# szabodabo/CUDA-MPI-Reductions

Hardware: AMD Instinct MI355X
Metric: reduction bandwidth (GB/s, whole node), 1B-double sum at 1/2/4/8 MI355X (higher is better)
Workload: dtype fp64; 1 GPU; global_batch=1000000000, seq_len=1, parallelism=dp1, backend=nccl, n_total_elements=1000000000, op=SUM, collective=fused, launch=graph (chunk 871, 1 replays)

## Files before the change

### csrc/kernels/direct.hip

```cpp
#include <hip/hip_runtime.h>

#include <algorithm>
#include <cstdint>
#include <cstring>

#include "mireduce/check.hpp"
#include "mireduce/device.hpp"
#include "mireduce/direct.hpp"
#include "mireduce/peer.hpp"
#include "mireduce/ops.hpp"

namespace mireduce {
namespace kern {

__device__ __forceinline__ void peer_barrier(const DirectDesc* d, int phase, unsigned e, unsigned err,
                                             bool release) {
  asm volatile("s_waitcnt vmcnt(0)" ::: "memory");
  __syncthreads();
  if (threadIdx.x < 64) {
    const int lane = threadIdx.x;
    if (release) __builtin_amdgcn_fence(__ATOMIC_RELEASE, "");
    const int world = d->world;
    const uint64_t slot = (static_cast<uint64_t>(phase) * kMaxDirectBlocks + blockIdx.x) * kMaxDirectRanks;
    if (lane < world) {
      __hip_atomic_store(d->sig[lane] + slot + d->rank, e, __ATOMIC_RELAXED, __HIP_MEMORY_SCOPE_SYSTEM);
      const unsigned* mine = d->sig[d->rank] + slot + lane;
      const uint64_t limit = err ? 0 : d->timeout_ticks;
      const uint64_t t0 = static_cast<uint64_t>(wall_clock64());
      while (__hip_atomic_load(mine, __ATOMIC_RELAXED, __HIP_MEMORY_SCOPE_SYSTEM) != e) {
        if (static_cast<uint64_t>(wall_clock64()) - t0 > limit) {
          __hip_atomic_fetch_or(d->ctl + 1, 1u, __ATOMIC_RELAXED, __HIP_MEMORY_SCOPE_AGENT);
          break;
        }
        __builtin_amdgcn_s_sleep(1);
      }
    }
    __builtin_amdgcn_fence(__ATOMIC_ACQUIRE, "");
  }
  __syncthreads();
}

__device__ __forceinline__ void block_range(uint64_t nvec, uint64_t* v0, uint64_t* v1) {
  const uint64_t per = (nvec + gridDim.x - 1) / gridDim.x;
  *v0 = std::min<uint64_t>(nvec, blockIdx.x * per);
  *v1 = std::min<uint64_t>(nvec, *v0 + per);
}

template <class T>
__device__ __forceinline__ uint64_t chunk_elems(uint64_t count, int world) {
  constexpr uint64_t N = 16 / sizeof(T);
  const uint64_t per = (count + world - 1) / world;
  return (per + N - 1) / N * N;
}

template <int W>
constexpr int direct_unroll() {
  return W >= 4 ? 1 : (W >= 2 ? 2 : 4);
}

template <class OpT, class T, int W>
__global__ __launch_bounds__(kDirectBlock) void direct_kernel(const DirectDesc* __restrict__ d, uint64_t count,
                                                               int gather_rank) {
  constexpr int N = 16 / sizeof(T);
  constexpr int U = W > 0 ? direct_unroll<W>() : 1;
  using V = T __attribute__((ext_vector_type(N)));
  __shared__ unsigned s_epoch, s_err;
  if (threadIdx.x == 0) {
    s_epoch = __hip_atomic_load(d->ctl, __ATOMIC_RELAXED, __HIP_MEMORY_SCOPE_AGENT) + 1u;
    s_err = __hip_atomic_load(d->ctl + 1, __ATOMIC_RELAXED, __HIP_MEMORY_SCOPE_AGENT);
  }
  __syncthreads();
  const unsigned e = s_epoch;
  const int world = W > 0 ? W : d->world;
  const int rank = d->rank;

  peer_barrier(d, 0, e, s_err, true);

  const uint64_t per = chunk_elems<T>(count, world);
  const uint64_t perv = per / N;
  uint64_t v0, v1;
  block_range(perv, &v0, &v1);
  {
    const uint64_t cb = std::min<uint64_t>(count, rank * per);
    const uint64_t ce = std::min<uint64_t>(count, cb + per);
    const uint64_t nvec = (ce - cb) / N;
    const uint64_t r1 = std::min(v1, nvec);
    T* out = reinterpret_cast<T*>(d->out[rank]);
    if constexpr (W > 0) {
      for (uint64_t i0 = v0 + threadIdx.x; i0 < r1; i0 += U * kDirectBlock) {
        V v[U][W];
#pragma unroll
        for (int u = 0; u < U; ++u) {
          const uint64_t i = i0 + static_cast<uint64_t>(u) * kDirectBlock;
          if (i < r1)
#pragma unroll
            for (int p = 0; p < W; ++p)
              v[u][p] = __builtin_nontemporal_load(reinterpret_cast<const V*>(d->in[p]) + cb / N + i);
        }
#pragma unroll
        for (int u = 0; u < U; ++u) {
          const uint64_t i = i0 + static_cast<uint64_t>(u) * kDirectBlock;
          if (i >= r1) continue;
          V acc = v[u][0];
#pragma unroll
          for (int p = 1; p < W; ++p)
#pragma unroll
            for (int k = 0; k < N; ++k) acc[k] = OpT::apply(acc[k], v[u][p][k]);
          reinterpret_cast<V*>(out)[cb / N + i] = acc;
        }
      }
    } else {
      for (uint64_t i = v0 + threadIdx.x; i < r1; i += kDirectBlock) {
        const uint64_t off = cb / N + i;
        V acc = __builtin_nontemporal_load(reinterpret_cast<const V*>(d->in[0]) + off);
        for (int p = 1; p < world; ++p) {
          const V v = __builtin_nontemporal_load(reinterpret_cast<const V*>(d->in[p]) + off);
#pragma unroll
          for (int k = 0; k < N; ++k) acc[k] = OpT::apply(acc[k], v[k]);
        }
        reinterpret_cast<V*>(out)[off] = acc;
      }
    }
    if (blockIdx.x == gridDim.x - 1) {
      for (uint64_t i = cb + nvec * N + threadIdx.x; i < ce; i += kDirectBlock) {
        T acc = reinterpret_cast<const T*>(d->in[0])[i];
        for (int p = 1; p < world; ++p) acc = OpT::apply(acc, reinterpret_cast<const T*>(d->in[p])[i]);
        out[i] = acc;
      }
    }
  }

  peer_barrier(d, 1, e, s_err, true);

  if (gather_rank < 0 || gather_rank == rank) {
    T* mine = reinterpret_cast<T*>(d->out[rank]);
    if constexpr (W > 0) {
      uint64_t nv[W];
#pragma unroll
      for (int p = 0; p < W; ++p) {
        const uint64_t b = std::min<uint64_t>(count, p * per);
        nv[p] = p == rank ? 0 : (std::min<uint64_t>(count, b + per) - b) / N;
      }
      for (uint64_t i0 = v0 + threadIdx.x; i0 < v1; i0 += U * kDirectBlock) {
        V v[U][W];
#pragma unroll
        for (int u = 0; u < U; ++u) {
          const uint64_t i = i0 + static_cast<uint64_t>(u) * kDirectBlock;
#pragma unroll
          for (int p = 0; p < W; ++p)
            if (i < v1 && i < nv[p])
              v[u][p] = __builtin_nontemporal_load(reinterpret_cast<const V*>(d->out[p]) + p * perv + i);
        }
#pragma unroll
        for (int u = 0; u < U; ++u) {
          const uint64_t i = i0 + static_cast<uint64_t>(u) * kDirectBlock;
#pragma unroll
          for (int p = 0; p < W; ++p)
            if (i < v1 && i < nv[p]) reinterpret_cast<V*>(mine)[p * perv + i] = v[u][p];
        }
      }
    } else {
      for (int p = 0; p < world; ++p) {
        if (p == rank) continue;
        const uint64_t b = std::min<uint64_t>(count, p * per);
        const uint64_t n = (std::min<uint64_t>(count, b + per) - b) / N;
        const uint64_t e1 = std::min(v1, n);
        for (uint64_t i = v0 + threadIdx.x; i < e1; i += kDirectBlock)
          reinterpret_cast<V*>(mine)[p * perv + i] = __builtin_nontemporal_load(reinterpret_cast<const V*>(d->out[p]) + p * perv + i);
      }
    }
    if (blockIdx.x == gridDim.x - 1) {
      for (int p = 0; p < world; ++p) {
        if (p == rank) continue;
        const uint64_t b = std::min<uint64_t>(count, p * per);
        const uint64_t e1 = std::min<uint64_t>(count, b + per);
        for (uint64_t i = b + (e1 - b) / N * N + threadIdx.x; i < e1; i += kDirectBlock)
          mine[i] = reinterpret_cast<const T*>(d->out[p])[i];
      }
    }
  }

  peer_barrier(d, 2, e, s_err, false);
  if (threadIdx.x == 0) {
    const unsigned prev = __hip_atomic_fetch_add(d->ctl + 2, 1u, __ATOMIC_RELAXED, __HIP_MEMORY_SCOPE_AGENT);
    if (prev == gridDim.x - 1) {
      __hip_atomic_store(d->ctl + 2, 0u, __ATOMIC_RELAXED, __HIP_MEMORY_SCOPE_AGENT);
      __hip_atomic_store(d->ctl, e, __ATOMIC_RELAXED, __HIP_MEMORY_SCOPE_AGENT);
    }
  }
}

}

void direct_chunk(size_t count, size_t elem_size, int world, int r, size_t* begin, size_t* end) {
  const size_t vec = 16 / elem_size;
  size_t per = (count + world - 1) / world;
  per = (per + vec - 1) / vec * vec;
  *begin = std::min(count, static_cast<size_t>(r) * per);
  *end = std::min(count, static_cast<size_t>(r + 1) * per);
}

namespace {

constexpr size_t kSigBytes = static_cast<size_t>(kDirectPhases) * kMaxDirectBlocks * kMaxDirectRanks * sizeof(unsigned);

using DirectFn = void (*)(const DirectDesc*, uint64_t, int, int, hipStream_t);

template <class OpT, class T, int W>
void launch_w(const DirectDesc* d, uint64_t count, int gather, int grid, hipStream_t s) {
  hipLaunchKernelGGL((kern::direct_kernel<OpT, T, W>), dim3(grid), dim3(kDirectBlock), 0, s, d, count, gather);
}

template <class OpT, class T>
DirectFn pick_world(int world) {
  switch (world) {
    case 1: return launch_w<OpT, T, 1>;
    case 2: return launch_w<OpT, T, 2>;
    case 3: return launch_w<OpT, T, 3>;
    case 4: return launch_w<OpT, T, 4>;
    case 5: return launch_w<OpT, T, 5>;
    case 6: return launch_w<OpT, T, 6>;
    case 7: return launch_w<OpT, T, 7>;
    case 8: return launch_w<OpT, T, 8>;
    default: return launch_w<OpT, T, 0>;
  }
}

template <class OpT>
DirectFn pick_type(DType t, int world) {
  switch (t) {
    case DType::Int32: return pick_world<OpT, int32_t>(world);
    case DType::Int64: return pick_world<OpT, int64_t>(world);
    case DType::Float32: return pick_world<OpT, float>(world);
    case DType::Float64: return pick_world<OpT, double>(world);
    default: MIREDUCE_REQUIRE(false, "direct: int32, int64, float32 or float64 only");
  }
  return nullptr;
}

}

DirectAllreduce::DirectAllreduce(int device, size_t bytes, int grid, double timeout_s) : timeout_s_(timeout_s) {
  MIREDUCE_REQUIRE(timeout_s > 0, "direct: timeout must be positive");
  if (device < 0) MIREDUCE_HIP_THROW(hipGetDevice(&device));
  device_ = device;
  DeviceGuard g(device_);
  grid_ = grid > 0 ? grid : device_cus(device_);
  MIREDUCE_REQUIRE(grid_ <= kMaxDirectBlocks, "direct: grid exceeds kMaxDirectBlocks");
  bytes_ = (std::max<size_t>(bytes, 16) + 255) / 256 * 256;
  MIREDUCE_HIP_THROW(hipExtMallocWithFlags(&in_, bytes_, hipDeviceMallocFinegrained));
  MIREDUCE_HIP_THROW(hipExtMallocWithFlags(&out_, bytes_, hipDeviceMallocFinegrained));
  MIREDUCE_HIP_THROW(hipExtMallocWithFlags(reinterpret_cast<void**>(&sig_), kSigBytes, hipDeviceMallocUncached));
  MIREDUCE_HIP_THROW(hipMemset(sig_, 0, kSigBytes));
  MIREDUCE_HIP_THROW(hipMalloc(reinterpret_cast<void**>(&ctl_), 256));
  MIREDUCE_HIP_THROW(hipMemset(ctl_, 0, 256));
  MIREDUCE_HIP_THROW(hipMalloc(reinterpret_cast<void**>(&desc_), sizeof(DirectDesc)));
  MIREDUCE_HIP_THROW(hipDeviceSynchronize());
}

DirectAllreduce::~DirectAllreduce() {
  DeviceGuard g(device_);
  for (void* p : opened_) (void)hipIpcCloseMemHandle(p);
  (void)hipFree(sink_);
  (void)hipFree(desc_);
  (void)hipFree(ctl_);
  (void)hipFree(sig_);
  (void)hipFree(out_);
  (void)hipFree(in_);
  (void)hipGetLastError();
}

std::vector<char> DirectAllreduce::handles() const {
  std::vector<char> h(kHandleBytes);
  void* bufs[3] = {in_, out_, sig_};
  for (int k = 0; k < 3; ++k) {
    hipIpcMemHandle_t m;
    MIREDUCE_HIP_THROW(hipIpcGetMemHandle(&m, bufs[k]));
    std::memcpy(h.data() + k * sizeof(IpcHandleBytes), &m, sizeof m);
  }
  const int32_t gr = grid_;
  std::memcpy(h.data() + 3 * sizeof(IpcHandleBytes), &gr, sizeof gr);
  return h;
}

void DirectAllreduce::connect(int rank, int world, const std::vector<std::vector<char>>& all) {
  MIREDUCE_REQUIRE(!connected_, "direct: already connected");
  MIREDUCE_REQUIRE(world >= 1 && world <= kMaxDirectRanks, "direct: world must be 1..16");
  MIREDUCE_REQUIRE(rank >= 0 && rank < world, "direct: rank out of range");
  MIREDUCE_REQUIRE(all.size() == static_cast<size_t>(world), "direct: one handle set per rank");
  DeviceGuard g(device_);
  DirectDesc d{};
  for (int r = 0; r < world; ++r) {
    MIREDUCE_REQUIRE(all[r].size() == kHandleBytes, "direct: bad handle size");
    int32_t gr = 0;
    std::memcpy(&gr, all[r].data() + 3 * sizeof(IpcHandleBytes), sizeof gr);
    MIREDUCE_REQUIRE(gr == grid_, "direct: every rank must use the same grid");
    if (r == rank) {
      d.in[r] = static_cast<const char*>(in_);
      d.out[r] = static_cast<char*>(out_);
      d.sig[r] = sig_;
      continue;
    }
    void* p[3] = {nullptr, nullptr, nullptr};
    for (int k = 0; k < 3; ++k) {
      hipIpcMemHandle_t m;
      std::memcpy(&m, all[r].data() + k * sizeof(IpcHandleBytes), sizeof m);
      MIREDUCE_HIP_THROW(hipIpcOpenMemHandle(&p[k], m, hipIpcMemLazyEnablePeerAccess));
      opened_.push_back(p[k]);
    }
    d.in[r] = static_cast<const char*>(p[0]);
    peer_in_.push_back(p[0]);
    d.out[r] = static_cast<char*>(p[1]);
    d.sig[r] = static_cast<unsigned*>(p[2]);
  }
  d.ctl = ctl_;
  d.rank = rank;
  d.world = world;
  int khz = 0;
  if (hipDeviceGetAttribute(&khz, hipDeviceAttributeWallClockRate, device_) != hipSuccess || khz <= 0) khz = 100000;
  d.timeout_ticks = static_cast<uint64_t>(timeout_s_ * 1e3 * khz);
  MIREDUCE_HIP_THROW(hipMemcpy(desc_, &d, sizeof d, hipMemcpyHostToDevice));
  MIREDUCE_HIP_THROW(hipDeviceSynchronize());
  rank_ = rank;
  world_ = world;
  connected_ = true;
}

void DirectAllreduce::launch(size_t count, DType t, Op op, int gather_rank, hipStream_t s) {
  MIREDUCE_REQUIRE(connected_, "direct: connect() first");
  MIREDUCE_REQUIRE(count * dtype_size(t) <= bytes_, "direct: count exceeds the registered buffers");
  DirectFn fn = nullptr;
  switch (op) {
    case Op::Sum: fn = pick_type<SumOp>(t, world_); break;
    case Op::Min: fn = pick_type<MinOp>(t, world_); break;
    case Op::Max: fn = pick_type<MaxOp>(t, world_); break;
    default: MIREDUCE_REQUIRE(false, "direct: SUM, MIN or MAX");
  }
  (void)hipGetLastError();
  fn(desc_, count, gather_rank, grid_, s);
  MIREDUCE_HIP_THROW(hipGetLastError());
}

void DirectAllreduce::allreduce(size_t count, DType t, Op op, hipStream_t s) { launch(count, t, op, -1, s); }

void DirectAllreduce::reduce(size_t count, DType t, Op op, int root, hipStream_t s) {
  MIREDUCE_REQUIRE(root >= 0 && root < world_, "direct: root out of range");
  launch(count, t, op, root, s);
}

void DirectAllreduce::read_peers(size_t bytes_each, hipStream_t s) {
  MIREDUCE_REQUIRE(connected_, "direct: connect() first");
  MIREDUCE_REQUIRE(bytes_each <= bytes_, "direct: read_peers beyond the registered buffers");
  DeviceGuard g(device_);
  PeerSources src{};
  int n = 0;
  if (peer_in_.empty()) src.p[n++] = in_;
  for (const void* p : peer_in_) src.p[n++] = p;
  const int grid = 128 * n;
  if (!sink_) MIREDUCE_HIP_THROW(hipMalloc(reinterpret_cast<void**>(&sink_), 128 * kMaxPeerSources * sizeof(uint32_t)));
  peer_read(src, n, bytes_each, sink_, grid, s);
}

unsigned DirectAllreduce::error() const {
  unsigned v = 0;
  DeviceGuard g(device_);
  MIREDUCE_HIP_THROW(hipMemcpy(&v, ctl_ + 1, sizeof v, hipMemcpyDeviceToHost));
  return v;
}

unsigned DirectAllreduce::epoch() const {
  unsigned v = 0;
  DeviceGuard g(device_);
  MIREDUCE_HIP_THROW(hipMemcpy(&v, ctl_, sizeof v, hipMemcpyDeviceToHost));
  return v;
}

}
```

Before: 7359 GB/s.

## Software-pipeline direct reduce and gather loops with global nontemporal tiles; skip barriers at world 1

Rewrites the reduce-scatter and gather phases of the direct kernel so that full tiles go through a double-buffered load/store loop. It uses explicit global address-space nontemporal loads and stores and places sched barriers so the next tile's loads are issued before the current tile's stores. This replaces flat, predicated, vmcnt(0)-serialised accesses. For a single rank it drops all three peer barriers and the gather phase. Range helpers move into a shared header, and reference assembly dumps are added. Risks are extra register pressure at large world sizes and nontemporal stores changing cache behaviour for readers of the output.

```diff
diff --git a/csrc/kernels/direct.hip b/csrc/kernels/direct.hip
--- a/csrc/kernels/direct.hip
+++ b/csrc/kernels/direct.hip
@@ -9,6 +9,8 @@
 #include "mireduce/direct.hpp"
 #include "mireduce/peer.hpp"
 #include "mireduce/ops.hpp"
+
+#include "direct_ranges.hpp"
 
 namespace mireduce {
 namespace kern {
@@ -40,22 +42,50 @@
   __syncthreads();
 }
 
-__device__ __forceinline__ void block_range(uint64_t nvec, uint64_t* v0, uint64_t* v1) {
-  const uint64_t per = (nvec + gridDim.x - 1) / gridDim.x;
-  *v0 = std::min<uint64_t>(nvec, blockIdx.x * per);
-  *v1 = std::min<uint64_t>(nvec, *v0 + per);
-}
-
-template <class T>
-__device__ __forceinline__ uint64_t chunk_elems(uint64_t count, int world) {
-  constexpr uint64_t N = 16 / sizeof(T);
-  const uint64_t per = (count + world - 1) / world;
-  return (per + N - 1) / N * N;
-}
-
 template <int W>
 constexpr int direct_unroll() {
   return W >= 4 ? 1 : (W >= 2 ? 2 : 4);
+}
+
+template <class V>
+using GlobalPtr = V __attribute__((address_space(1)))*;
+
+template <class V>
+__device__ __forceinline__ V ld_global_nt(const char* base, uint32_t off) {
+  return __builtin_nontemporal_load((GlobalPtr<const V>)(base + off));
+}
+template <class V>
+__device__ __forceinline__ void st_global(char* base, uint32_t off, V v) {
+  __builtin_nontemporal_store(v, (GlobalPtr<V>)(base + off));
+}
+
+template <class Set, class Load, class Store>
+__device__ __forceinline__ void stream_full_tiles(uint64_t nfull, Load load, Store store) {
+  if (nfull == 0) return;
+  __builtin_amdgcn_s_waitcnt(0);
+  Set a, b;
+  load(a, uint64_t{0});
+  uint64_t k = 0;
+#pragma clang loop unroll(disable)
+  for (; k + 2 < nfull; k += 2) {
+    load(b, k + 1);
+    __builtin_amdgcn_sched_barrier(0);
+    store(a, k);
+    __builtin_amdgcn_sched_barrier(0);
+    load(a, k + 2);
+    __builtin_amdgcn_sched_barrier(0);
+    store(b, k + 1);
+    __builtin_amdgcn_sched_barrier(0);
+  }
+  if (k + 1 < nfull) {
+    load(b, k + 1);
+    __builtin_amdgcn_sched_barrier(0);
+    store(a, k);
+    __builtin_amdgcn_sched_barrier(0);
+    store(b, k + 1);
+  } else {
+    store(a, k);
+  }
 }
 
 template <class OpT, class T, int W>
@@ -63,7 +93,10 @@
                                                                int gather_rank) {
   constexpr int N = 16 / sizeof(T);
   constexpr int U = W > 0 ? direct_unroll<W>() : 1;
+  constexpr int UT = direct_ranges::tile_unroll(W);
+  constexpr uint64_t kTile = static_cast<uint64_t>(kDirectBlock) * UT;
   using V = T __attribute__((ext_vector_type(N)));
+  namespace dr = direct_ranges;
   __shared__ unsigned s_epoch, s_err;
   if (threadIdx.x == 0) {
     s_epoch = __hip_atomic_load(d->ctl, __ATOMIC_RELAXED, __HIP_MEMORY_SCOPE_AGENT) + 1u;
@@ -74,20 +107,48 @@
   const int world = W > 0 ? W : d->world;
   const int rank = d->rank;
 
-  peer_barrier(d, 0, e, s_err, true);
-
-  const uint64_t per = chunk_elems<T>(count, world);
+  if constexpr (W != 1) peer_barrier(d, 0, e, s_err, true);
+
+  const uint64_t per = dr::chunk_elems(count, world, sizeof(T));
   const uint64_t perv = per / N;
   uint64_t v0, v1;
-  block_range(perv, &v0, &v1);
+  dr::block_range(perv, gridDim.x, blockIdx.x, &v0, &v1);
   {
-    const uint64_t cb = std::min<uint64_t>(count, rank * per);
-    const uint64_t ce = std::min<uint64_t>(count, cb + per);
+    uint64_t cb, ce;
+    dr::chunk_bounds(count, per, rank, &cb, &ce);
     const uint64_t nvec = (ce - cb) / N;
     const uint64_t r1 = std::min(v1, nvec);
     T* out = reinterpret_cast<T*>(d->out[rank]);
     if constexpr (W > 0) {
-      for (uint64_t i0 = v0 + threadIdx.x; i0 < r1; i0 += U * kDirectBlock) {
+      const dr::TileSplit ts = dr::tile_split(v0, r1, kTile);
+      struct Set {
+        V v[UT][W];
+      };
+      const char* src[W];
+#pragma unroll
+      for (int p = 0; p < W; ++p) src[p] = d->in[p] + (cb / N + v0) * 16;
+      char* dst = d->out[rank] + (cb / N + v0) * 16;
+      stream_full_tiles<Set>(
+          ts.nfull,
+          [&](Set& s, uint64_t k) {
+#pragma unroll
+            for (int u = 0; u < UT; ++u)
+#pragma unroll
+              for (int p = 0; p < W; ++p)
+                s.v[u][p] = ld_global_nt<V>(src[p] + k * (kTile * 16), dr::tile_lane_bytes(u, threadIdx.x, kDirectBlock));
+          },
+          [&](Set& s, uint64_t k) {
+#pragma unroll
+            for (int u = 0; u < UT; ++u) {
+              V acc = s.v[u][0];
+#pragma unroll
+              for (int p = 1; p < W; ++p)
+#pragma unroll
+                for (int j = 0; j < N; ++j) acc[j] = OpT::apply(acc[j], s.v[u][p][j]);
+              st_global<V>(dst + k * (kTile * 16), dr::tile_lane_bytes(u, threadIdx.x, kDirectBlock), acc);
+            }
+          });
+      for (uint64_t i0 = ts.rem0 + threadIdx.x; i0 < r1; i0 += U * kDirectBlock) {
         V v[U][W];
 #pragma unroll
         for (int u = 0; u < U; ++u) {
@@ -130,18 +191,47 @@
     }
   }
 
-  peer_barrier(d, 1, e, s_err, true);
-
-  if (gather_rank < 0 || gather_rank == rank) {
+  if constexpr (W != 1) peer_barrier(d, 1, e, s_err, true);
+
+  if (W != 1 && (gather_rank < 0 || gather_rank == rank)) {
     T* mine = reinterpret_cast<T*>(d->out[rank]);
-    if constexpr (W > 0) {
+    if constexpr (W > 1) {
+      const uint64_t g1 = dr::gather_common_end(count, per, N, W, rank, v1);
+      const dr::TileSplit ts = dr::tile_split(v0, g1, kTile);
+      struct Set {
+        V v[UT][W - 1];
+      };
+      const char* src[W - 1];
+      char* dst[W - 1];
+#pragma unroll
+      for (int q = 0; q < W - 1; ++q) {
+        const int p = q + (q >= rank ? 1 : 0);
+        src[q] = d->out[p] + (p * perv + v0) * 16;
+        dst[q] = d->out[rank] + (p * perv + v0) * 16;
+      }
+      stream_full_tiles<Set>(
+          ts.nfull,
+          [&](Set& s, uint64_t k) {
+#pragma unroll
+            for (int u = 0; u < UT; ++u)
+#pragma unroll
+              for (int q = 0; q < W - 1; ++q)
+                s.v[u][q] = ld_global_nt<V>(src[q] + k * (kTile * 16), dr::tile_lane_bytes(u, threadIdx.x, kDirectBlock));
+          },
+          [&](Set& s, uint64_t k) {
+#pragma unroll
+            for (int u = 0; u < UT; ++u)
+#pragma unroll
+              for (int q = 0; q < W - 1; ++q)
+                st_global<V>(dst[q] + k * (kTile * 16), dr::tile_lane_bytes(u, threadIdx.x, kDirectBlock), s.v[u][q]);
+          });
       uint64_t nv[W];
 #pragma unroll
       for (int p = 0; p < W; ++p) {
         const uint64_t b = std::min<uint64_t>(count, p * per);
         nv[p] = p == rank ? 0 : (std::min<uint64_t>(count, b + per) - b) / N;
       }
-      for (uint64_t i0 = v0 + threadIdx.x; i0 < v1; i0 += U * kDirectBlock) {
+      for (uint64_t i0 = ts.rem0 + threadIdx.x; i0 < v1; i0 += U * kDirectBlock) {
         V v[U][W];
 #pragma unroll
         for (int u = 0; u < U; ++u) {
@@ -180,7 +270,7 @@
     }
   }
 
-  peer_barrier(d, 2, e, s_err, false);
+  if constexpr (W != 1) peer_barrier(d, 2, e, s_err, false);
   if (threadIdx.x == 0) {
     const unsigned prev = __hip_atomic_fetch_add(d->ctl + 2, 1u, __ATOMIC_RELAXED, __HIP_MEMORY_SCOPE_AGENT);
     if (prev == gridDim.x - 1) {
@@ -193,11 +283,10 @@
 }
 
 void direct_chunk(size_t count, size_t elem_size, int world, int r, size_t* begin, size_t* end) {
-  const size_t vec = 16 / elem_size;
-  size_t per = (count + world - 1) / world;
-  per = (per + vec - 1) / vec * vec;
-  *begin = std::min(count, static_cast<size_t>(r) * per);
-  *end = std::min(count, static_cast<size_t>(r + 1) * per);
+  uint64_t b, e;
+  direct_ranges::chunk_bounds(count, direct_ranges::chunk_elems(count, world, elem_size), r, &b, &e);
+  *begin = b;
+  *end = e;
 }
 
 namespace {
diff --git a/csrc/kernels/direct_ranges.hpp b/csrc/kernels/direct_ranges.hpp
--- /dev/null
+++ b/csrc/kernels/direct_ranges.hpp
@@ -0,0 +1,61 @@
+#pragma once
+
+#include <cstdint>
+
+#include "mireduce/ops.hpp"
+
+namespace mireduce {
+namespace direct_ranges {
+
+MIREDUCE_HD uint64_t min_u64(uint64_t a, uint64_t b) { return a < b ? a : b; }
+
+MIREDUCE_HD uint64_t chunk_elems(uint64_t count, int world, uint64_t elem_size) {
+  const uint64_t n = 16 / elem_size;
+  const uint64_t per = (count + world - 1) / world;
+  return (per + n - 1) / n * n;
+}
+
+MIREDUCE_HD void chunk_bounds(uint64_t count, uint64_t per, int r, uint64_t* begin, uint64_t* end) {
+  *begin = min_u64(count, static_cast<uint64_t>(r) * per);
+  *end = min_u64(count, *begin + per);
+}
+
+MIREDUCE_HD void block_range(uint64_t nvec, uint32_t grid, uint32_t block, uint64_t* v0, uint64_t* v1) {
+  const uint64_t per = (nvec + grid - 1) / grid;
+  *v0 = min_u64(nvec, block * per);
+  *v1 = min_u64(nvec, *v0 + per);
+}
+
+struct TileSplit {
+  uint64_t nfull;
+  uint64_t rem0;
+};
+
+MIREDUCE_HD constexpr int tile_unroll(int world) { return world == 1 ? 2 : 1; }
+
+MIREDUCE_HD constexpr uint32_t tile_lane_bytes(uint32_t u, uint32_t tid, uint32_t block) {
+  return (u * block + tid) * 16u;
+}
+
+MIREDUCE_HD TileSplit tile_split(uint64_t v0, uint64_t r1, uint64_t tile) {
+  const uint64_t n = r1 > v0 ? r1 - v0 : 0;
+  TileSplit s;
+  s.nfull = n / tile;
+  s.rem0 = v0 + s.nfull * tile;
+  return s;
+}
+
+MIREDUCE_HD uint64_t gather_common_end(uint64_t count, uint64_t per, uint64_t vec_elems, int world, int rank,
+                                       uint64_t v1) {
+  uint64_t e = v1;
+  for (int p = 0; p < world; ++p) {
+    if (p == rank) continue;
+    uint64_t b, c;
+    chunk_bounds(count, per, p, &b, &c);
+    e = min_u64(e, (c - b) / vec_elems);
+  }
+  return e;
+}
+
+}
+}
diff --git a/profiles/direct_stream/loops_after_double_sum_w1.s b/profiles/direct_stream/loops_after_double_sum_w1.s
--- /dev/null
+++ b/profiles/direct_stream/loops_after_double_sum_w1.s
@@ -0,0 +1,112 @@
+
+.LBB27_8:
+	s_mov_b64 s[34:35], s[28:29]
+	s_lshl_b64 s[28:29], s[28:29], 14
+	s_or_b32 s38, s28, 0x4000
+	s_mov_b32 s39, s29
+	v_lshl_add_u64 v[28:29], v[12:13], 0, s[38:39]
+	v_add_co_u32_e32 v30, vcc, 0x2000, v28
+	s_nop 1
+	v_addc_co_u32_e32 v31, vcc, 0, v29, vcc
+	global_load_dwordx4 v[18:21], v[28:29], off nt
+	global_load_dwordx4 v[24:27], v[30:31], off nt
+	v_lshl_add_u64 v[28:29], v[14:15], 0, s[28:29]
+	s_waitcnt vmcnt(3)
+	global_store_dwordx4 v[28:29], v[6:9], off nt
+	s_nop 1
+	v_add_co_u32_e32 v6, vcc, 0x2000, v28
+	s_nop 1
+	v_addc_co_u32_e32 v7, vcc, 0, v29, vcc
+	s_waitcnt vmcnt(3)
+	global_store_dwordx4 v[6:7], v[2:5], off nt
+	s_lshl_b64 s[28:29], s[30:31], 14
+	v_lshl_add_u64 v[28:29], v[12:13], 0, s[28:29]
+	v_add_co_u32_e32 v30, vcc, 0x2000, v28
+	s_nop 1
+	v_addc_co_u32_e32 v31, vcc, 0, v29, vcc
+	global_load_dwordx4 v[6:9], v[28:29], off nt
+	global_load_dwordx4 v[2:5], v[30:31], off nt
+	v_lshl_add_u64 v[28:29], v[14:15], 0, s[38:39]
+	s_waitcnt vmcnt(5)
+	global_store_dwordx4 v[28:29], v[18:21], off nt
+	s_nop 1
+	v_add_co_u32_e32 v18, vcc, 0x2000, v28
+	s_nop 1
+	v_addc_co_u32_e32 v19, vcc, 0, v29, vcc
+	s_waitcnt vmcnt(5)
+	global_store_dwordx4 v[18:19], v[24:27], off nt
+	s_add_u32 s30, s30, 2
+	s_addc_u32 s31, s31, 0
+	s_add_u32 s28, s34, 2
+	s_addc_u32 s29, s35, 0
+	s_add_u32 s34, s34, 4
+	s_addc_u32 s35, s35, 0
+	v_cmp_lt_u64_e32 vcc, s[34:35], v[16:17]
+	s_cbranch_vccnz .LBB27_8
+
+.LBB27_17:
+	s_or_b64 exec, exec, s[0:1]
+	v_lshl_add_u64 v[18:19], v[18:19], 0, s[40:41]
+	v_cmp_le_u64_e32 vcc, s[22:23], v[18:19]
+	s_or_b64 s[30:31], vcc, s[30:31]
+	s_andn2_b64 exec, exec, s[30:31]
+	s_cbranch_execz .LBB27_30
+.LBB27_18:
+	v_lshl_add_u64 v[20:21], v[18:19], 4, s[28:29]
+	flat_load_dwordx4 v[14:17], v[20:21] nt
+	v_lshl_add_u64 v[24:25], v[18:19], 0, s[34:35]
+	v_cmp_gt_u64_e64 s[0:1], s[22:23], v[24:25]
+	s_and_saveexec_b64 s[4:5], s[0:1]
+	s_cbranch_execz .LBB27_20
+	v_add_co_u32_e32 v2, vcc, 0x2000, v20
+	s_nop 1
+	v_addc_co_u32_e32 v3, vcc, 0, v21, vcc
+	flat_load_dwordx4 v[2:5], v[2:3] nt
+.LBB27_20:
+	s_or_b64 exec, exec, s[4:5]
+	v_lshl_add_u64 v[24:25], v[18:19], 0, s[36:37]
+	v_cmp_gt_u64_e64 s[4:5], s[22:23], v[24:25]
+	s_and_saveexec_b64 s[6:7], s[4:5]
+	s_cbranch_execz .LBB27_22
+	v_add_co_u32_e32 v6, vcc, 0x4000, v20
+	s_nop 1
+	v_addc_co_u32_e32 v7, vcc, 0, v21, vcc
+	flat_load_dwordx4 v[6:9], v[6:7] nt
+.LBB27_22:
+	s_or_b64 exec, exec, s[6:7]
+	v_lshl_add_u64 v[24:25], v[18:19], 0, s[38:39]
+	v_cmp_gt_u64_e64 s[6:7], s[22:23], v[24:25]
+	s_and_saveexec_b64 s[42:43], s[6:7]
+	s_cbranch_execz .LBB27_24
+	v_add_co_u32_e32 v10, vcc, 0x6000, v20
+	s_nop 1
+	v_addc_co_u32_e32 v11, vcc, 0, v21, vcc
+	flat_load_dwordx4 v[10:13], v[10:11] nt
+.LBB27_24:
+	s_or_b64 exec, exec, s[42:43]
+	v_lshl_add_u64 v[20:21], v[18:19], 4, s[26:27]
+	s_waitcnt vmcnt(0) lgkmcnt(0)
+	flat_store_dwordx4 v[20:21], v[14:17]
+	s_and_saveexec_b64 s[42:43], s[0:1]
+	s_cbranch_execnz .LBB27_27
+	s_or_b64 exec, exec, s[42:43]
+	s_and_saveexec_b64 s[0:1], s[4:5]
+	s_cbranch_execnz .LBB27_28
+.LBB27_26:
+	s_or_b64 exec, exec, s[0:1]
+	s_and_saveexec_b64 s[0:1], s[6:7]
+	s_cbranch_execz .LBB27_17
+
+.LBB27_26:
+	s_or_b64 exec, exec, s[0:1]
+	s_and_saveexec_b64 s[0:1], s[6:7]
+	s_cbranch_execz .LBB27_17
+	s_branch .LBB27_29
+.LBB27_27:
+	v_add_co_u32_e32 v14, vcc, 0x2000, v20
+	s_nop 1
+	v_addc_co_u32_e32 v15, vcc, 0, v21, vcc
+	flat_store_dwordx4 v[14:15], v[2:5]
+	s_or_b64 exec, exec, s[42:43]
+	s_and_saveexec_b64 s[0:1], s[4:5]
+	s_cbranch_execz .LBB27_26
diff --git a/profiles/direct_stream/loops_after_double_sum_w8.s b/profiles/direct_stream/loops_after_double_sum_w8.s
--- /dev/null
+++ b/profiles/direct_stream/loops_after_double_sum_w8.s
@@ -0,0 +1,736 @@
+
+.LBB34_20:
+	s_lshl_b64 s[2:3], s[18:19], 13
+	s_mov_b64 s[22:23], s[18:19]
+	s_or_b32 s18, s2, 0x2000
+	s_mov_b32 s19, s3
+	v_lshl_add_u64 v[58:59], v[34:35], 0, s[18:19]
+	v_lshl_add_u64 v[62:63], v[36:37], 0, s[18:19]
+	v_lshl_add_u64 v[66:67], v[42:43], 0, s[18:19]
+	v_lshl_add_u64 v[70:71], v[44:45], 0, s[18:19]
+	v_lshl_add_u64 v[74:75], v[46:47], 0, s[18:19]
+	v_lshl_add_u64 v[78:79], v[48:49], 0, s[18:19]
+	v_lshl_add_u64 v[82:83], v[50:51], 0, s[18:19]
+	v_lshl_add_u64 v[86:87], v[52:53], 0, s[18:19]
+	global_load_dwordx4 v[58:61], v[58:59], off nt
+	s_nop 0
+	global_load_dwordx4 v[62:65], v[62:63], off nt
+	s_nop 0
+	global_load_dwordx4 v[66:69], v[66:67], off nt
+	s_nop 0
+	global_load_dwordx4 v[70:73], v[70:71], off nt
+	s_nop 0
+	global_load_dwordx4 v[74:77], v[74:75], off nt
+	s_nop 0
+	global_load_dwordx4 v[78:81], v[78:79], off nt
+	s_nop 0
+	global_load_dwordx4 v[82:85], v[82:83], off nt
+	s_nop 0
+	global_load_dwordx4 v[86:89], v[86:87], off nt
+	s_waitcnt vmcnt(14)
+	v_add_f64 v[26:27], v[26:27], v[30:31]
+	v_add_f64 v[28:29], v[28:29], v[32:33]
+	s_waitcnt vmcnt(13)
+	v_add_f64 v[22:23], v[22:23], v[26:27]
+	v_add_f64 v[24:25], v[24:25], v[28:29]
+	s_waitcnt vmcnt(12)
+	v_add_f64 v[18:19], v[18:19], v[22:23]
+	v_add_f64 v[20:21], v[20:21], v[24:25]
+	s_waitcnt vmcnt(11)
+	v_add_f64 v[14:15], v[14:15], v[18:19]
+	v_add_f64 v[16:17], v[16:17], v[20:21]
+	s_waitcnt vmcnt(10)
+	v_add_f64 v[10:11], v[10:11], v[14:15]
+	v_add_f64 v[12:13], v[12:13], v[16:17]
+	s_waitcnt vmcnt(9)
+	v_add_f64 v[6:7], v[6:7], v[10:11]
+	v_add_f64 v[8:9], v[8:9], v[12:13]
+	s_waitcnt vmcnt(8)
+	v_add_f64 v[2:3], v[2:3], v[6:7]
+	v_add_f64 v[4:5], v[4:5], v[8:9]
+	v_lshl_add_u64 v[6:7], v[54:55], 0, s[2:3]
+	global_store_dwordx4 v[6:7], v[2:5], off nt
+	s_lshl_b64 s[2:3], s[20:21], 13
+	s_nop 0
+	v_lshl_add_u64 v[2:3], v[34:35], 0, s[2:3]
+	global_load_dwordx4 v[26:29], v[2:3], off nt
+	v_lshl_add_u64 v[2:3], v[36:37], 0, s[2:3]
+	global_load_dwordx4 v[30:33], v[2:3], off nt
+	v_lshl_add_u64 v[2:3], v[42:43], 0, s[2:3]
+	global_load_dwordx4 v[22:25], v[2:3], off nt
+	v_lshl_add_u64 v[2:3], v[44:45], 0, s[2:3]
+	global_load_dwordx4 v[18:21], v[2:3], off nt
+	v_lshl_add_u64 v[2:3], v[46:47], 0, s[2:3]
+	global_load_dwordx4 v[14:17], v[2:3], off nt
+	v_lshl_add_u64 v[2:3], v[48:49], 0, s[2:3]
+	global_load_dwordx4 v[10:13], v[2:3], off nt
+	v_lshl_add_u64 v[2:3], v[50:51], 0, s[2:3]
+	global_load_dwordx4 v[6:9], v[2:3], off nt
+	v_lshl_add_u64 v[2:3], v[52:53], 0, s[2:3]
+	global_load_dwordx4 v[2:5], v[2:3], off nt
+	s_waitcnt vmcnt(15)
+	v_add_f64 v[58:59], v[58:59], v[62:63]
+	v_add_f64 v[60:61], v[60:61], v[64:65]
+	s_waitcnt vmcnt(14)
+	v_add_f64 v[58:59], v[58:59], v[66:67]
+	v_add_f64 v[60:61], v[60:61], v[68:69]
+	s_waitcnt vmcnt(13)
+	v_add_f64 v[58:59], v[58:59], v[70:71]
+	v_add_f64 v[60:61], v[60:61], v[72:73]
+	s_waitcnt vmcnt(12)
+	v_add_f64 v[58:59], v[58:59], v[74:75]
+	v_add_f64 v[60:61], v[60:61], v[76:77]
+	s_waitcnt vmcnt(11)
+	v_add_f64 v[58:59], v[58:59], v[78:79]
+	v_add_f64 v[60:61], v[60:61], v[80:81]
+	s_waitcnt vmcnt(10)
+	v_add_f64 v[58:59], v[58:59], v[82:83]
+	v_add_f64 v[60:61], v[60:61], v[84:85]
+	s_waitcnt vmcnt(9)
+	v_add_f64 v[58:59], v[58:59], v[86:87]
+	v_add_f64 v[60:61], v[60:61], v[88:89]
+	v_lshl_add_u64 v[62:63], v[54:55], 0, s[18:19]
+	global_store_dwordx4 v[62:63], v[58:61], off nt
+	s_add_u32 s20, s20, 2
+	s_addc_u32 s21, s21, 0
+	s_add_u32 s18, s22, 2
+	s_addc_u32 s19, s23, 0
+	s_add_u32 s2, s22, 4
+	s_addc_u32 s3, s23, 0
+	v_cmp_lt_u64_e32 vcc, s[2:3], v[56:57]
+	s_cbranch_vccnz .LBB34_20
+
+.LBB34_29:
+	v_lshlrev_b64 v[28:29], 4, v[2:3]
+	v_lshl_add_u64 v[4:5], s[8:9], 0, v[28:29]
+	v_lshl_add_u64 v[8:9], s[10:11], 0, v[28:29]
+	v_lshl_add_u64 v[12:13], s[12:13], 0, v[28:29]
+	v_lshl_add_u64 v[16:17], s[14:15], 0, v[28:29]
+	v_lshl_add_u64 v[20:21], s[16:17], 0, v[28:29]
+	v_lshl_add_u64 v[24:25], s[18:19], 0, v[28:29]
+	v_lshl_add_u64 v[32:33], s[20:21], 0, v[28:29]
+	v_lshl_add_u64 v[36:37], s[2:3], 0, v[28:29]
+	flat_load_dwordx4 v[4:7], v[4:5] nt
+	s_nop 0
+	flat_load_dwordx4 v[8:11], v[8:9] nt
+	s_nop 0
+	flat_load_dwordx4 v[12:15], v[12:13] nt
+	s_nop 0
+	flat_load_dwordx4 v[16:19], v[16:17] nt
+	s_nop 0
+	flat_load_dwordx4 v[20:23], v[20:21] nt
+	s_nop 0
+	flat_load_dwordx4 v[24:27], v[24:25] nt
+	s_nop 0
+	flat_load_dwordx4 v[32:35], v[32:33] nt
+	s_nop 0
+	flat_load_dwordx4 v[40:43], v[36:37] nt
+	v_lshl_add_u64 v[2:3], v[2:3], 0, s[22:23]
+	v_cmp_le_u64_e32 vcc, s[38:39], v[2:3]
+	v_lshl_add_u64 v[28:29], s[6:7], 0, v[28:29]
+	s_or_b64 s[4:5], vcc, s[4:5]
+	s_waitcnt vmcnt(0) lgkmcnt(0)
+	v_add_f64 v[4:5], v[4:5], v[8:9]
+	v_add_f64 v[6:7], v[6:7], v[10:11]
+	v_add_f64 v[4:5], v[4:5], v[12:13]
+	v_add_f64 v[6:7], v[6:7], v[14:15]
+	v_add_f64 v[4:5], v[4:5], v[16:17]
+	v_add_f64 v[6:7], v[6:7], v[18:19]
+	v_add_f64 v[4:5], v[4:5], v[20:21]
+	v_add_f64 v[6:7], v[6:7], v[22:23]
+	v_add_f64 v[4:5], v[4:5], v[24:25]
+	v_add_f64 v[6:7], v[6:7], v[26:27]
+	v_add_f64 v[4:5], v[4:5], v[32:33]
+	v_add_f64 v[6:7], v[6:7], v[34:35]
+	v_add_f64 v[4:5], v[4:5], v[40:41]
+	v_add_f64 v[6:7], v[6:7], v[42:43]
+	flat_store_dwordx4 v[28:29], v[4:7]
+	s_andn2_b64 exec, exec, s[4:5]
+	s_cbranch_execnz .LBB34_29
+
+.LBB34_67:
+	s_mov_b64 s[2:3], s[78:79]
+	s_lshl_b64 s[78:79], s[78:79], 13
+	s_or_b32 s82, s78, 0x2000
+	s_mov_b32 s83, s79
+	v_lshl_add_u64 v[66:67], v[34:35], 0, s[82:83]
+	v_lshl_add_u64 v[70:71], v[36:37], 0, s[82:83]
+	v_lshl_add_u64 v[74:75], v[40:41], 0, s[82:83]
+	v_lshl_add_u64 v[78:79], v[42:43], 0, s[82:83]
+	v_lshl_add_u64 v[82:83], v[44:45], 0, s[82:83]
+	v_lshl_add_u64 v[86:87], v[46:47], 0, s[82:83]
+	v_lshl_add_u64 v[90:91], v[48:49], 0, s[82:83]
+	global_load_dwordx4 v[66:69], v[66:67], off nt
+	s_nop 0
+	global_load_dwordx4 v[70:73], v[70:71], off nt
+	s_nop 0
+	global_load_dwordx4 v[74:77], v[74:75], off nt
+	s_nop 0
+	global_load_dwordx4 v[78:81], v[78:79], off nt
+	s_nop 0
+	global_load_dwordx4 v[82:85], v[82:83], off nt
+	s_nop 0
+	global_load_dwordx4 v[86:89], v[86:87], off nt
+	s_nop 0
+	global_load_dwordx4 v[90:93], v[90:91], off nt
+	v_lshl_add_u64 v[94:95], v[50:51], 0, s[78:79]
+	s_waitcnt vmcnt(13)
+	global_store_dwordx4 v[94:95], v[26:29], off nt
+	s_nop 1
+	v_lshl_add_u64 v[26:27], v[52:53], 0, s[78:79]
+	s_waitcnt vmcnt(13)
+	global_store_dwordx4 v[26:27], v[22:25], off nt
+	s_nop 1
+	v_lshl_add_u64 v[22:23], v[54:55], 0, s[78:79]
+	s_waitcnt vmcnt(13)
+	global_store_dwordx4 v[22:23], v[18:21], off nt
+	s_nop 1
+	v_lshl_add_u64 v[18:19], v[56:57], 0, s[78:79]
+	s_waitcnt vmcnt(13)
+	global_store_dwordx4 v[18:19], v[14:17], off nt
+	s_nop 1
+	v_lshl_add_u64 v[14:15], v[58:59], 0, s[78:79]
+	s_waitcnt vmcnt(13)
+	global_store_dwordx4 v[14:15], v[10:13], off nt
+	s_nop 1
+	v_lshl_add_u64 v[10:11], v[60:61], 0, s[78:79]
+	s_waitcnt vmcnt(13)
+	global_store_dwordx4 v[10:11], v[6:9], off nt
+	s_nop 1
+	v_lshl_add_u64 v[6:7], v[62:63], 0, s[78:79]
+	s_waitcnt vmcnt(13)
+	global_store_dwordx4 v[6:7], v[2:5], off nt
+	s_lshl_b64 s[78:79], s[4:5], 13
+	s_nop 0
+	v_lshl_add_u64 v[2:3], v[34:35], 0, s[78:79]
+	global_load_dwordx4 v[26:29], v[2:3], off nt
+	v_lshl_add_u64 v[2:3], v[36:37], 0, s[78:79]
+	global_load_dwordx4 v[22:25], v[2:3], off nt
+	v_lshl_add_u64 v[2:3], v[40:41], 0, s[78:79]
+	global_load_dwordx4 v[18:21], v[2:3], off nt
+	v_lshl_add_u64 v[2:3], v[42:43], 0, s[78:79]
+	global_load_dwordx4 v[14:17], v[2:3], off nt
+	v_lshl_add_u64 v[2:3], v[44:45], 0, s[78:79]
+	global_load_dwordx4 v[10:13], v[2:3], off nt
+	v_lshl_add_u64 v[2:3], v[46:47], 0, s[78:79]
+	global_load_dwordx4 v[6:9], v[2:3], off nt
+	v_lshl_add_u64 v[2:3], v[48:49], 0, s[78:79]
+	global_load_dwordx4 v[2:5], v[2:3], off nt
+	v_lshl_add_u64 v[94:95], v[50:51], 0, s[82:83]
+	s_waitcnt vmcnt(20)
+	global_store_dwordx4 v[94:95], v[66:69], off nt
+	s_nop 1
+	v_lshl_add_u64 v[66:67], v[52:53], 0, s[82:83]
+	s_waitcnt vmcnt(20)
+	global_store_dwordx4 v[66:67], v[70:73], off nt
+	v_lshl_add_u64 v[66:67], v[54:55], 0, s[82:83]
+	s_waitcnt vmcnt(20)
+	global_store_dwordx4 v[66:67], v[74:77], off nt
+	v_lshl_add_u64 v[66:67], v[56:57], 0, s[82:83]
+	s_waitcnt vmcnt(20)
+	global_store_dwordx4 v[66:67], v[78:81], off nt
+	v_lshl_add_u64 v[66:67], v[58:59], 0, s[82:83]
+	s_waitcnt vmcnt(20)
+	global_store_dwordx4 v[66:67], v[82:85], off nt
+	v_lshl_add_u64 v[66:67], v[60:61], 0, s[82:83]
+	s_waitcnt vmcnt(20)
+	global_store_dwordx4 v[66:67], v[86:89], off nt
+	v_lshl_add_u64 v[66:67], v[62:63], 0, s[82:83]
+	s_waitcnt vmcnt(20)
+	global_store_dwordx4 v[66:67], v[90:93], off nt
+	s_add_u32 s4, s4, 2
+	s_addc_u32 s5, s5, 0
+	s_add_u32 s78, s2, 2
+	s_addc_u32 s79, s3, 0
+	s_add_u32 s2, s2, 4
+	s_addc_u32 s3, s3, 0
+	v_cmp_lt_u64_e32 vcc, s[2:3], v[64:65]
+	s_cbranch_vccnz .LBB34_67
+
+.LBB34_75:
+	s_or_b64 exec, exec, s[2:3]
+	s_mov_b64 s[2:3], 0x200
+	v_lshl_add_u64 v[34:35], v[34:35], 0, s[2:3]
+	v_cmp_le_u64_e32 vcc, s[30:31], v[34:35]
+	s_or_b64 s[94:95], vcc, s[94:95]
+	s_andn2_b64 exec, exec, s[94:95]
+	s_cbranch_execz .LBB34_108
+.LBB34_76:
+	v_cmp_gt_u64_e32 vcc, s[72:73], v[34:35]
+	s_and_b64 s[96:97], s[22:23], vcc
+	s_and_saveexec_b64 s[2:3], s[96:97]
+	s_cbranch_execz .LBB34_78
+	s_load_dwordx2 s[4:5], s[24:25], 0x80
+	s_waitcnt vmcnt(0) lgkmcnt(0)
+	v_lshl_add_u64 v[14:15], v[34:35], 4, s[4:5]
+	flat_load_dwordx4 v[14:17], v[14:15] nt
+.LBB34_78:
+	s_or_b64 exec, exec, s[2:3]
+	v_cmp_gt_u64_e32 vcc, s[50:51], v[34:35]
+	s_and_b64 s[98:99], s[20:21], vcc
+	s_and_saveexec_b64 s[2:3], s[98:99]
+	s_cbranch_execz .LBB34_80
+	s_load_dwordx2 s[4:5], s[24:25], 0x88
+	s_lshl_b64 s[6:7], s[26:27], 4
+	s_waitcnt lgkmcnt(0)
+	s_add_u32 s4, s4, s6
+	s_addc_u32 s5, s5, s7
+	s_waitcnt vmcnt(0)
+	v_lshl_add_u64 v[30:31], v[34:35], 4, s[4:5]
+	flat_load_dwordx4 v[30:33], v[30:31] nt
+.LBB34_80:
+	s_or_b64 exec, exec, s[2:3]
+	v_cmp_gt_u64_e32 vcc, s[52:53], v[34:35]
+	s_and_b64 s[6:7], s[18:19], vcc
+	s_and_saveexec_b64 s[2:3], s[6:7]
+	s_cbranch_execz .LBB34_82
+	s_load_dwordx2 s[4:5], s[24:25], 0x90
+	s_lshl_b64 s[38:39], s[28:29], 4
+	s_waitcnt lgkmcnt(0)
+	s_add_u32 s4, s4, s38
+	s_addc_u32 s5, s5, s39
+	s_waitcnt vmcnt(0)
+	v_lshl_add_u64 v[26:27], v[34:35], 4, s[4:5]
+	flat_load_dwordx4 v[26:29], v[26:27] nt
+.LBB34_82:
+	s_or_b64 exec, exec, s[2:3]
+	v_cmp_gt_u64_e32 vcc, s[74:75], v[34:35]
+	s_and_b64 s[4:5], s[16:17], vcc
+	s_and_saveexec_b64 s[2:3], s[4:5]
+	s_cbranch_execz .LBB34_84
+	s_load_dwordx2 s[38:39], s[24:25], 0x98
+	s_waitcnt lgkmcnt(0)
+	s_add_u32 s38, s38, s84
+	s_addc_u32 s39, s39, s85
+	s_waitcnt vmcnt(0)
+	v_lshl_add_u64 v[22:23], v[34:35], 4, s[38:39]
+	flat_load_dwordx4 v[22:25], v[22:23] nt
+.LBB34_84:
+	s_or_b64 exec, exec, s[2:3]
+	v_cmp_gt_u64_e32 vcc, s[76:77], v[34:35]
+	s_and_b64 s[38:39], s[14:15], vcc
+	s_and_saveexec_b64 s[2:3], s[38:39]
+	s_cbranch_execz .LBB34_86
+	s_load_dwordx2 s[40:41], s[24:25], 0xa0
+	s_waitcnt lgkmcnt(0)
+	s_add_u32 s40, s40, s86
+	s_addc_u32 s41, s41, s87
+	s_waitcnt vmcnt(0)
+	v_lshl_add_u64 v[18:19], v[34:35], 4, s[40:41]
+	flat_load_dwordx4 v[18:21], v[18:19] nt
+.LBB34_86:
+	s_or_b64 exec, exec, s[2:3]
+	v_cmp_gt_u64_e32 vcc, s[78:79], v[34:35]
+	s_and_b64 s[40:41], s[12:13], vcc
+	s_and_saveexec_b64 s[2:3], s[40:41]
+	s_cbranch_execz .LBB34_88
+	s_load_dwordx2 s[44:45], s[24:25], 0xa8
+	s_waitcnt lgkmcnt(0)
+	s_add_u32 s44, s44, s88
+	s_addc_u32 s45, s45, s89
+	s_waitcnt vmcnt(0)
+	v_lshl_add_u64 v[10:11], v[34:35], 4, s[44:45]
+	flat_load_dwordx4 v[10:13], v[10:11] nt
+.LBB34_88:
+	s_or_b64 exec, exec, s[2:3]
+	v_cmp_gt_u64_e32 vcc, s[80:81], v[34:35]
+	s_and_b64 s[2:3], s[10:11], vcc
+	s_and_saveexec_b64 vcc, s[2:3]
+	s_cbranch_execz .LBB34_90
+	s_load_dwordx2 s[44:45], s[24:25], 0xb0
+	s_waitcnt lgkmcnt(0)
+	s_add_u32 s44, s44, s90
+	s_addc_u32 s45, s45, s91
+	s_waitcnt vmcnt(0)
+	v_lshl_add_u64 v[6:7], v[34:35], 4, s[44:45]
+	flat_load_dwordx4 v[6:9], v[6:7] nt
+.LBB34_90:
+	s_or_b64 exec, exec, vcc
+	v_cmp_gt_u64_e32 vcc, s[82:83], v[34:35]
+	s_and_b64 vcc, s[8:9], vcc
+	s_and_saveexec_b64 s[44:45], vcc
+	s_cbranch_execnz .LBB34_99
+	s_or_b64 exec, exec, s[44:45]
+	s_waitcnt lgkmcnt(0)
+	v_lshl_add_u64 v[36:37], v[34:35], 4, s[0:1]
+	s_and_saveexec_b64 s[44:45], s[96:97]
+	s_cbranch_execnz .LBB34_100
+.LBB34_92:
+	s_or_b64 exec, exec, s[44:45]
+	s_and_saveexec_b64 s[44:45], s[98:99]
+	s_cbranch_execnz .LBB34_101
+.LBB34_93:
+	s_or_b64 exec, exec, s[44:45]
+	s_and_saveexec_b64 s[44:45], s[6:7]
+	s_cbranch_execnz .LBB34_102
+.LBB34_94:
+	s_or_b64 exec, exec, s[44:45]
+	s_and_saveexec_b64 s[6:7], s[4:5]
+	s_cbranch_execnz .LBB34_103
+.LBB34_95:
+	s_or_b64 exec, exec, s[6:7]
+	s_and_saveexec_b64 s[4:5], s[38:39]
+	s_cbranch_execnz .LBB34_104
+.LBB34_96:
+	s_or_b64 exec, exec, s[4:5]
+	s_and_saveexec_b64 s[4:5], s[40:41]
+	s_cbranch_execnz .LBB34_105
+.LBB34_97:
+	s_or_b64 exec, exec, s[4:5]
+	s_and_saveexec_b64 s[4:5], s[2:3]
+	s_cbranch_execnz .LBB34_106
+.LBB34_98:
+	s_or_b64 exec, exec, s[4:5]
+	s_and_saveexec_b64 s[2:3], vcc
+	s_cbranch_execz .LBB34_75
+
+.LBB34_92:
+	s_or_b64 exec, exec, s[44:45]
+	s_and_saveexec_b64 s[44:45], s[98:99]
+	s_cbranch_execnz .LBB34_101
+.LBB34_93:
+	s_or_b64 exec, exec, s[44:45]
+	s_and_saveexec_b64 s[44:45], s[6:7]
+	s_cbranch_execnz .LBB34_102
+.LBB34_94:
+	s_or_b64 exec, exec, s[44:45]
+	s_and_saveexec_b64 s[6:7], s[4:5]
+	s_cbranch_execnz .LBB34_103
+.LBB34_95:
+	s_or_b64 exec, exec, s[6:7]
+	s_and_saveexec_b64 s[4:5], s[38:39]
+	s_cbranch_execnz .LBB34_104
+.LBB34_96:
+	s_or_b64 exec, exec, s[4:5]
+	s_and_saveexec_b64 s[4:5], s[40:41]
+	s_cbranch_execnz .LBB34_105
+.LBB34_97:
+	s_or_b64 exec, exec, s[4:5]
+	s_and_saveexec_b64 s[4:5], s[2:3]
+	s_cbranch_execnz .LBB34_106
+.LBB34_98:
+	s_or_b64 exec, exec, s[4:5]
+	s_and_saveexec_b64 s[2:3], vcc
+	s_cbranch_execz .LBB34_75
+	s_branch .LBB34_107
+.LBB34_99:
+	s_load_dwordx2 s[46:47], s[24:25], 0xb8
+	s_waitcnt lgkmcnt(0)
+	s_add_u32 s46, s46, s92
+	s_addc_u32 s47, s47, s93
+	s_waitcnt vmcnt(0)
+	v_lshl_add_u64 v[2:3], v[34:35], 4, s[46:47]
+	flat_load_dwordx4 v[2:5], v[2:3] nt
+	s_or_b64 exec, exec, s[44:45]
+	v_lshl_add_u64 v[36:37], v[34:35], 4, s[0:1]
+	s_and_saveexec_b64 s[44:45], s[96:97]
+	s_cbranch_execz .LBB34_92
+
+.LBB34_93:
+	s_or_b64 exec, exec, s[44:45]
+	s_and_saveexec_b64 s[44:45], s[6:7]
+	s_cbranch_execnz .LBB34_102
+.LBB34_94:
+	s_or_b64 exec, exec, s[44:45]
+	s_and_saveexec_b64 s[6:7], s[4:5]
+	s_cbranch_execnz .LBB34_103
+.LBB34_95:
+	s_or_b64 exec, exec, s[6:7]
+	s_and_saveexec_b64 s[4:5], s[38:39]
+	s_cbranch_execnz .LBB34_104
+.LBB34_96:
+	s_or_b64 exec, exec, s[4:5]
+	s_and_saveexec_b64 s[4:5], s[40:41]
+	s_cbranch_execnz .LBB34_105
+.LBB34_97:
+	s_or_b64 exec, exec, s[4:5]
+	s_and_saveexec_b64 s[4:5], s[2:3]
+	s_cbranch_execnz .LBB34_106
+.LBB34_98:
+	s_or_b64 exec, exec, s[4:5]
+	s_and_saveexec_b64 s[2:3], vcc
+	s_cbranch_execz .LBB34_75
+	s_branch .LBB34_107
+.LBB34_99:
+	s_load_dwordx2 s[46:47], s[24:25], 0xb8
+	s_waitcnt lgkmcnt(0)
+	s_add_u32 s46, s46, s92
+	s_addc_u32 s47, s47, s93
+	s_waitcnt vmcnt(0)
+	v_lshl_add_u64 v[2:3], v[34:35], 4, s[46:47]
+	flat_load_dwordx4 v[2:5], v[2:3] nt
+	s_or_b64 exec, exec, s[44:45]
+	v_lshl_add_u64 v[36:37], v[34:35], 4, s[0:1]
+	s_and_saveexec_b64 s[44:45], s[96:97]
+	s_cbranch_execz .LBB34_92
+.LBB34_100:
+	s_waitcnt vmcnt(0)
+	flat_store_dwordx4 v[36:37], v[14:17]
+	s_or_b64 exec, exec, s[44:45]
+	s_and_saveexec_b64 s[44:45], s[98:99]
+	s_cbranch_execz .LBB34_93
+
+.LBB34_94:
+	s_or_b64 exec, exec, s[44:45]
+	s_and_saveexec_b64 s[6:7], s[4:5]
+	s_cbranch_execnz .LBB34_103
+.LBB34_95:
+	s_or_b64 exec, exec, s[6:7]
+	s_and_saveexec_b64 s[4:5], s[38:39]
+	s_cbranch_execnz .LBB34_104
+.LBB34_96:
+	s_or_b64 exec, exec, s[4:5]
+	s_and_saveexec_b64 s[4:5], s[40:41]
+	s_cbranch_execnz .LBB34_105
+.LBB34_97:
+	s_or_b64 exec, exec, s[4:5]
+	s_and_saveexec_b64 s[4:5], s[2:3]
+	s_cbranch_execnz .LBB34_106
+.LBB34_98:
+	s_or_b64 exec, exec, s[4:5]
+	s_and_saveexec_b64 s[2:3], vcc
+	s_cbranch_execz .LBB34_75
+	s_branch .LBB34_107
+.LBB34_99:
+	s_load_dwordx2 s[46:47], s[24:25], 0xb8
+	s_waitcnt lgkmcnt(0)
+	s_add_u32 s46, s46, s92
+	s_addc_u32 s47, s47, s93
+	s_waitcnt vmcnt(0)
+	v_lshl_add_u64 v[2:3], v[34:35], 4, s[46:47]
+	flat_load_dwordx4 v[2:5], v[2:3] nt
+	s_or_b64 exec, exec, s[44:45]
+	v_lshl_add_u64 v[36:37], v[34:35], 4, s[0:1]
+	s_and_saveexec_b64 s[44:45], s[96:97]
+	s_cbranch_execz .LBB34_92
+.LBB34_100:
+	s_waitcnt vmcnt(0)
+	flat_store_dwordx4 v[36:37], v[14:17]
+	s_or_b64 exec, exec, s[44:45]
+	s_and_saveexec_b64 s[44:45], s[98:99]
+	s_cbranch_execz .LBB34_93
+.LBB34_101:
+	v_lshl_add_u64 v[40:41], s[26:27], 4, v[36:37]
+	s_waitcnt vmcnt(0)
+	flat_store_dwordx4 v[40:41], v[30:33]
+	s_or_b64 exec, exec, s[44:45]
+	s_and_saveexec_b64 s[44:45], s[6:7]
+	s_cbranch_execz .LBB34_94
+
+.LBB34_95:
+	s_or_b64 exec, exec, s[6:7]
+	s_and_saveexec_b64 s[4:5], s[38:39]
+	s_cbranch_execnz .LBB34_104
+.LBB34_96:
+	s_or_b64 exec, exec, s[4:5]
+	s_and_saveexec_b64 s[4:5], s[40:41]
+	s_cbranch_execnz .LBB34_105
+.LBB34_97:
+	s_or_b64 exec, exec, s[4:5]
+	s_and_saveexec_b64 s[4:5], s[2:3]
+	s_cbranch_execnz .LBB34_106
+.LBB34_98:
+	s_or_b64 exec, exec, s[4:5]
+	s_and_saveexec_b64 s[2:3], vcc
+	s_cbranch_execz .LBB34_75
+	s_branch .LBB34_107
+.LBB34_99:
+	s_load_dwordx2 s[46:47], s[24:25], 0xb8
+	s_waitcnt lgkmcnt(0)
+	s_add_u32 s46, s46, s92
+	s_addc_u32 s47, s47, s93
+	s_waitcnt vmcnt(0)
+	v_lshl_add_u64 v[2:3], v[34:35], 4, s[46:47]
+	flat_load_dwordx4 v[2:5], v[2:3] nt
+	s_or_b64 exec, exec, s[44:45]
+	v_lshl_add_u64 v[36:37], v[34:35], 4, s[0:1]
+	s_and_saveexec_b64 s[44:45], s[96:97]
+	s_cbranch_execz .LBB34_92
+.LBB34_100:
+	s_waitcnt vmcnt(0)
+	flat_store_dwordx4 v[36:37], v[14:17]
+	s_or_b64 exec, exec, s[44:45]
+	s_and_saveexec_b64 s[44:45], s[98:99]
+	s_cbranch_execz .LBB34_93
+.LBB34_101:
+	v_lshl_add_u64 v[40:41], s[26:27], 4, v[36:37]
+	s_waitcnt vmcnt(0)
+	flat_store_dwordx4 v[40:41], v[30:33]
+	s_or_b64 exec, exec, s[44:45]
+	s_and_saveexec_b64 s[44:45], s[6:7]
+	s_cbranch_execz .LBB34_94
+.LBB34_102:
+	v_lshl_add_u64 v[40:41], s[28:29], 4, v[36:37]
+	s_waitcnt vmcnt(0)
+	flat_store_dwordx4 v[40:41], v[26:29]
+	s_or_b64 exec, exec, s[44:45]
+	s_and_saveexec_b64 s[6:7], s[4:5]
+	s_cbranch_execz .LBB34_95
+
+.LBB34_96:
+	s_or_b64 exec, exec, s[4:5]
+	s_and_saveexec_b64 s[4:5], s[40:41]
+	s_cbranch_execnz .LBB34_105
+.LBB34_97:
+	s_or_b64 exec, exec, s[4:5]
+	s_and_saveexec_b64 s[4:5], s[2:3]
+	s_cbranch_execnz .LBB34_106
+.LBB34_98:
+	s_or_b64 exec, exec, s[4:5]
+	s_and_saveexec_b64 s[2:3], vcc
+	s_cbranch_execz .LBB34_75
+	s_branch .LBB34_107
+.LBB34_99:
+	s_load_dwordx2 s[46:47], s[24:25], 0xb8
+	s_waitcnt lgkmcnt(0)
+	s_add_u32 s46, s46, s92
+	s_addc_u32 s47, s47, s93
+	s_waitcnt vmcnt(0)
+	v_lshl_add_u64 v[2:3], v[34:35], 4, s[46:47]
+	flat_load_dwordx4 v[2:5], v[2:3] nt
+	s_or_b64 exec, exec, s[44:45]
+	v_lshl_add_u64 v[36:37], v[34:35], 4, s[0:1]
+	s_and_saveexec_b64 s[44:45], s[96:97]
+	s_cbranch_execz .LBB34_92
+.LBB34_100:
+	s_waitcnt vmcnt(0)
+	flat_store_dwordx4 v[36:37], v[14:17]
+	s_or_b64 exec, exec, s[44:45]
+	s_and_saveexec_b64 s[44:45], s[98:99]
+	s_cbranch_execz .LBB34_93
+.LBB34_101:
+	v_lshl_add_u64 v[40:41], s[26:27], 4, v[36:37]
+	s_waitcnt vmcnt(0)
+	flat_store_dwordx4 v[40:41], v[30:33]
+	s_or_b64 exec, exec, s[44:45]
+	s_and_saveexec_b64 s[44:45], s[6:7]
+	s_cbranch_execz .LBB34_94
+.LBB34_102:
+	v_lshl_add_u64 v[40:41], s[28:29], 4, v[36:37]
+	s_waitcnt vmcnt(0)
+	flat_store_dwordx4 v[40:41], v[26:29]
+	s_or_b64 exec, exec, s[44:45]
+	s_and_saveexec_b64 s[6:7], s[4:5]
+	s_cbranch_execz .LBB34_95
+.LBB34_103:
+	v_lshl_add_u64 v[40:41], v[36:37], 0, s[84:85]
+	s_waitcnt vmcnt(0)
+	flat_store_dwordx4 v[40:41], v[22:25]
+	s_or_b64 exec, exec, s[6:7]
+	s_and_saveexec_b64 s[4:5], s[38:39]
+	s_cbranch_execz .LBB34_96
+
+.LBB34_97:
+	s_or_b64 exec, exec, s[4:5]
+	s_and_saveexec_b64 s[4:5], s[2:3]
+	s_cbranch_execnz .LBB34_106
+.LBB34_98:
+	s_or_b64 exec, exec, s[4:5]
+	s_and_saveexec_b64 s[2:3], vcc
+	s_cbranch_execz .LBB34_75
+	s_branch .LBB34_107
+.LBB34_99:
+	s_load_dwordx2 s[46:47], s[24:25], 0xb8
+	s_waitcnt lgkmcnt(0)
+	s_add_u32 s46, s46, s92
+	s_addc_u32 s47, s47, s93
+	s_waitcnt vmcnt(0)
+	v_lshl_add_u64 v[2:3], v[34:35], 4, s[46:47]
+	flat_load_dwordx4 v[2:5], v[2:3] nt
+	s_or_b64 exec, exec, s[44:45]
+	v_lshl_add_u64 v[36:37], v[34:35], 4, s[0:1]
+	s_and_saveexec_b64 s[44:45], s[96:97]
+	s_cbranch_execz .LBB34_92
+.LBB34_100:
+	s_waitcnt vmcnt(0)
+	flat_store_dwordx4 v[36:37], v[14:17]
+	s_or_b64 exec, exec, s[44:45]
+	s_and_saveexec_b64 s[44:45], s[98:99]
+	s_cbranch_execz .LBB34_93
+.LBB34_101:
+	v_lshl_add_u64 v[40:41], s[26:27], 4, v[36:37]
+	s_waitcnt vmcnt(0)
+	flat_store_dwordx4 v[40:41], v[30:33]
+	s_or_b64 exec, exec, s[44:45]
+	s_and_saveexec_b64 s[44:45], s[6:7]
+	s_cbranch_execz .LBB34_94
+.LBB34_102:
+	v_lshl_add_u64 v[40:41], s[28:29], 4, v[36:37]
+	s_waitcnt vmcnt(0)
+	flat_store_dwordx4 v[40:41], v[26:29]
+	s_or_b64 exec, exec, s[44:45]
+	s_and_saveexec_b64 s[6:7], s[4:5]
+	s_cbranch_execz .LBB34_95
+.LBB34_103:
+	v_lshl_add_u64 v[40:41], v[36:37], 0, s[84:85]
+	s_waitcnt vmcnt(0)
+	flat_store_dwordx4 v[40:41], v[22:25]
+	s_or_b64 exec, exec, s[6:7]
+	s_and_saveexec_b64 s[4:5], s[38:39]
+	s_cbranch_execz .LBB34_96
+.LBB34_104:
+	v_lshl_add_u64 v[40:41], v[36:37], 0, s[86:87]
+	s_waitcnt vmcnt(0)
+	flat_store_dwordx4 v[40:41], v[18:21]
+	s_or_b64 exec, exec, s[4:5]
+	s_and_saveexec_b64 s[4:5], s[40:41]
+	s_cbranch_execz .LBB34_97
+
+.LBB34_98:
+	s_or_b64 exec, exec, s[4:5]
+	s_and_saveexec_b64 s[2:3], vcc
+	s_cbranch_execz .LBB34_75
+	s_branch .LBB34_107
+.LBB34_99:
+	s_load_dwordx2 s[46:47], s[24:25], 0xb8
+	s_waitcnt lgkmcnt(0)
+	s_add_u32 s46, s46, s92
+	s_addc_u32 s47, s47, s93
+	s_waitcnt vmcnt(0)
+	v_lshl_add_u64 v[2:3], v[34:35], 4, s[46:47]
+	flat_load_dwordx4 v[2:5], v[2:3] nt
+	s_or_b64 exec, exec, s[44:45]
+	v_lshl_add_u64 v[36:37], v[34:35], 4, s[0:1]
+	s_and_saveexec_b64 s[44:45], s[96:97]
+	s_cbranch_execz .LBB34_92
+.LBB34_100:
+	s_waitcnt vmcnt(0)
+	flat_store_dwordx4 v[36:37], v[14:17]
+	s_or_b64 exec, exec, s[44:45]
+	s_and_saveexec_b64 s[44:45], s[98:99]
+	s_cbranch_execz .LBB34_93
+.LBB34_101:
+	v_lshl_add_u64 v[40:41], s[26:27], 4, v[36:37]
+	s_waitcnt vmcnt(0)
+	flat_store_dwordx4 v[40:41], v[30:33]
+	s_or_b64 exec, exec, s[44:45]
+	s_and_saveexec_b64 s[44:45], s[6:7]
+	s_cbranch_execz .LBB34_94
+.LBB34_102:
+	v_lshl_add_u64 v[40:41], s[28:29], 4, v[36:37]
+	s_waitcnt vmcnt(0)
+	flat_store_dwordx4 v[40:41], v[26:29]
+	s_or_b64 exec, exec, s[44:45]
+	s_and_saveexec_b64 s[6:7], s[4:5]
+	s_cbranch_execz .LBB34_95
+.LBB34_103:
+	v_lshl_add_u64 v[40:41], v[36:37], 0, s[84:85]
+	s_waitcnt vmcnt(0)
+	flat_store_dwordx4 v[40:41], v[22:25]
+	s_or_b64 exec, exec, s[6:7]
+	s_and_saveexec_b64 s[4:5], s[38:39]
+	s_cbranch_execz .LBB34_96
+.LBB34_104:
+	v_lshl_add_u64 v[40:41], v[36:37], 0, s[86:87]
+	s_waitcnt vmcnt(0)
+	flat_store_dwordx4 v[40:41], v[18:21]
+	s_or_b64 exec, exec, s[4:5]
+	s_and_saveexec_b64 s[4:5], s[40:41]
+	s_cbranch_execz .LBB34_97
+.LBB34_105:
+	v_lshl_add_u64 v[40:41], v[36:37], 0, s[88:89]
+	s_waitcnt vmcnt(0)
+	flat_store_dwordx4 v[40:41], v[10:13]
+	s_or_b64 exec, exec, s[4:5]
+	s_and_saveexec_b64 s[4:5], s[2:3]
+	s_cbranch_execz .LBB34_98
diff --git a/profiles/direct_stream/loops_before_double_sum_w1.s b/profiles/direct_stream/loops_before_double_sum_w1.s
--- /dev/null
+++ b/profiles/direct_stream/loops_before_double_sum_w1.s
@@ -0,0 +1,200 @@
+
+.LBB27_19:
+	s_or_b64 exec, exec, s[8:9]
+	v_lshl_add_u64 v[22:23], v[22:23], 0, s[54:55]
+	v_cmp_le_u64_e32 vcc, s[34:35], v[22:23]
+	s_or_b64 s[46:47], vcc, s[46:47]
+	s_andn2_b64 exec, exec, s[46:47]
+	s_cbranch_execz .LBB27_32
+.LBB27_20:
+	v_lshl_add_u64 v[26:27], v[22:23], 4, s[44:45]
+	flat_load_dwordx4 v[14:17], v[26:27] nt
+	v_lshl_add_u64 v[28:29], v[22:23], 0, s[48:49]
+	v_cmp_gt_u64_e64 s[8:9], s[34:35], v[28:29]
+	s_and_saveexec_b64 s[10:11], s[8:9]
+	s_cbranch_execz .LBB27_22
+	v_lshl_add_u64 v[2:3], s[40:41], 4, v[24:25]
+	v_lshl_add_u64 v[2:3], v[28:29], 4, v[2:3]
+	flat_load_dwordx4 v[2:5], v[2:3] nt
+.LBB27_22:
+	s_or_b64 exec, exec, s[10:11]
+	v_lshl_add_u64 v[28:29], v[22:23], 0, s[50:51]
+	v_cmp_gt_u64_e64 s[10:11], s[34:35], v[28:29]
+	s_and_saveexec_b64 s[12:13], s[10:11]
+	s_cbranch_execz .LBB27_24
+	v_lshl_add_u64 v[6:7], s[40:41], 4, v[24:25]
+	v_lshl_add_u64 v[6:7], v[28:29], 4, v[6:7]
+	flat_load_dwordx4 v[6:9], v[6:7] nt
+.LBB27_24:
+	s_or_b64 exec, exec, s[12:13]
+	v_lshl_add_u64 v[28:29], v[22:23], 0, s[52:53]
+	v_cmp_gt_u64_e64 s[12:13], s[34:35], v[28:29]
+	s_and_saveexec_b64 s[56:57], s[12:13]
+	s_cbranch_execz .LBB27_26
+	v_add_co_u32_e32 v10, vcc, 0x6000, v26
+	v_mov_b64_e32 v[24:25], s[38:39]
+	s_nop 0
+	v_addc_co_u32_e32 v11, vcc, 0, v27, vcc
+	flat_load_dwordx4 v[10:13], v[10:11] nt
+.LBB27_26:
+	s_or_b64 exec, exec, s[56:57]
+	v_lshl_add_u64 v[26:27], v[22:23], 4, s[42:43]
+	s_waitcnt vmcnt(0) lgkmcnt(0)
+	flat_store_dwordx4 v[26:27], v[14:17]
+	s_and_saveexec_b64 s[56:57], s[8:9]
+	s_cbranch_execnz .LBB27_29
+	s_or_b64 exec, exec, s[56:57]
+	s_and_saveexec_b64 s[8:9], s[10:11]
+	s_cbranch_execnz .LBB27_30
+.LBB27_28:
+	s_or_b64 exec, exec, s[8:9]
+	s_and_saveexec_b64 s[8:9], s[12:13]
+	s_cbranch_execz .LBB27_19
+
+.LBB27_28:
+	s_or_b64 exec, exec, s[8:9]
+	s_and_saveexec_b64 s[8:9], s[12:13]
+	s_cbranch_execz .LBB27_19
+	s_branch .LBB27_31
+.LBB27_29:
+	v_add_co_u32_e32 v14, vcc, 0x2000, v26
+	s_nop 1
+	v_addc_co_u32_e32 v15, vcc, 0, v27, vcc
+	flat_store_dwordx4 v[14:15], v[2:5]
+	s_or_b64 exec, exec, s[56:57]
+	s_and_saveexec_b64 s[8:9], s[10:11]
+	s_cbranch_execz .LBB27_28
+
+.LBB27_53:
+	s_or_b64 exec, exec, s[0:1]
+	v_lshl_add_u64 v[20:21], v[26:27], 0, s[34:35]
+	v_cmp_le_u64_e32 vcc, s[22:23], v[20:21]
+	s_or_b64 s[30:31], vcc, s[30:31]
+	s_andn2_b64 exec, exec, s[30:31]
+	s_cbranch_execz .LBB27_70
+.LBB27_54:
+	v_cmp_gt_u64_e32 vcc, s[28:29], v[20:21]
+	s_and_saveexec_b64 s[0:1], vcc
+	s_cbranch_execz .LBB27_56
+	s_load_dwordx2 s[8:9], s[14:15], 0x80
+	s_waitcnt vmcnt(0) lgkmcnt(0)
+	v_lshl_add_u64 v[2:3], v[20:21], 4, s[8:9]
+	flat_load_dwordx4 v[2:5], v[2:3] nt
+.LBB27_56:
+	s_or_b64 exec, exec, s[0:1]
+	v_lshl_add_u64 v[22:23], v[20:21], 0, s[34:35]
+	v_cmp_gt_u64_e64 s[0:1], s[28:29], v[22:23]
+	s_and_saveexec_b64 s[8:9], s[0:1]
+	s_cbranch_execz .LBB27_58
+	s_load_dwordx2 s[10:11], s[14:15], 0x80
+	s_waitcnt vmcnt(0) lgkmcnt(0)
+	v_lshl_add_u64 v[6:7], v[22:23], 4, s[10:11]
+	flat_load_dwordx4 v[6:9], v[6:7] nt
+.LBB27_58:
+	s_or_b64 exec, exec, s[8:9]
+	v_lshl_add_u64 v[26:27], v[22:23], 0, s[34:35]
+	v_lshl_add_u64 v[24:25], v[20:21], 0, s[36:37]
+	v_cmp_gt_u64_e64 s[8:9], s[28:29], v[26:27]
+	s_and_saveexec_b64 s[10:11], s[8:9]
+	s_cbranch_execz .LBB27_60
+	s_load_dwordx2 s[40:41], s[14:15], 0x80
+	s_waitcnt vmcnt(0) lgkmcnt(0)
+	v_lshl_add_u64 v[10:11], v[24:25], 4, s[40:41]
+	flat_load_dwordx4 v[10:13], v[10:11] nt
+.LBB27_60:
+	s_or_b64 exec, exec, s[10:11]
+	v_lshl_add_u64 v[26:27], v[26:27], 0, s[34:35]
+	v_lshl_add_u64 v[28:29], v[20:21], 0, s[38:39]
+	v_cmp_gt_u64_e64 s[10:11], s[28:29], v[26:27]
+	s_and_saveexec_b64 s[40:41], s[10:11]
+	s_cbranch_execnz .LBB27_65
+	s_or_b64 exec, exec, s[40:41]
+	s_and_saveexec_b64 s[40:41], vcc
+	s_cbranch_execnz .LBB27_66
+.LBB27_62:
+	s_or_b64 exec, exec, s[40:41]
+	s_and_saveexec_b64 s[40:41], s[0:1]
+	s_cbranch_execnz .LBB27_67
+.LBB27_63:
+	s_or_b64 exec, exec, s[40:41]
+	s_and_saveexec_b64 s[0:1], s[8:9]
+	s_cbranch_execnz .LBB27_68
+.LBB27_64:
+	s_or_b64 exec, exec, s[0:1]
+	s_and_saveexec_b64 s[0:1], s[10:11]
+	s_cbranch_execz .LBB27_53
+
+.LBB27_62:
+	s_or_b64 exec, exec, s[40:41]
+	s_and_saveexec_b64 s[40:41], s[0:1]
+	s_cbranch_execnz .LBB27_67
+.LBB27_63:
+	s_or_b64 exec, exec, s[40:41]
+	s_and_saveexec_b64 s[0:1], s[8:9]
+	s_cbranch_execnz .LBB27_68
+.LBB27_64:
+	s_or_b64 exec, exec, s[0:1]
+	s_and_saveexec_b64 s[0:1], s[10:11]
+	s_cbranch_execz .LBB27_53
+	s_branch .LBB27_69
+.LBB27_65:
+	s_load_dwordx2 s[42:43], s[14:15], 0x80
+	s_waitcnt vmcnt(0) lgkmcnt(0)
+	v_lshl_add_u64 v[14:15], v[28:29], 4, s[42:43]
+	flat_load_dwordx4 v[14:17], v[14:15] nt
+	s_or_b64 exec, exec, s[40:41]
+	s_and_saveexec_b64 s[40:41], vcc
+	s_cbranch_execz .LBB27_62
+
+.LBB27_63:
+	s_or_b64 exec, exec, s[40:41]
+	s_and_saveexec_b64 s[0:1], s[8:9]
+	s_cbranch_execnz .LBB27_68
+.LBB27_64:
+	s_or_b64 exec, exec, s[0:1]
+	s_and_saveexec_b64 s[0:1], s[10:11]
+	s_cbranch_execz .LBB27_53
+	s_branch .LBB27_69
+.LBB27_65:
+	s_load_dwordx2 s[42:43], s[14:15], 0x80
+	s_waitcnt vmcnt(0) lgkmcnt(0)
+	v_lshl_add_u64 v[14:15], v[28:29], 4, s[42:43]
+	flat_load_dwordx4 v[14:17], v[14:15] nt
+	s_or_b64 exec, exec, s[40:41]
+	s_and_saveexec_b64 s[40:41], vcc
+	s_cbranch_execz .LBB27_62
+.LBB27_66:
+	v_lshl_add_u64 v[20:21], v[20:21], 4, s[24:25]
+	s_waitcnt vmcnt(0) lgkmcnt(0)
+	flat_store_dwordx4 v[20:21], v[2:5]
+	s_or_b64 exec, exec, s[40:41]
+	s_and_saveexec_b64 s[40:41], s[0:1]
+	s_cbranch_execz .LBB27_63
+
+.LBB27_64:
+	s_or_b64 exec, exec, s[0:1]
+	s_and_saveexec_b64 s[0:1], s[10:11]
+	s_cbranch_execz .LBB27_53
+	s_branch .LBB27_69
+.LBB27_65:
+	s_load_dwordx2 s[42:43], s[14:15], 0x80
+	s_waitcnt vmcnt(0) lgkmcnt(0)
+	v_lshl_add_u64 v[14:15], v[28:29], 4, s[42:43]
+	flat_load_dwordx4 v[14:17], v[14:15] nt
+	s_or_b64 exec, exec, s[40:41]
+	s_and_saveexec_b64 s[40:41], vcc
+	s_cbranch_execz .LBB27_62
+.LBB27_66:
+	v_lshl_add_u64 v[20:21], v[20:21], 4, s[24:25]
+	s_waitcnt vmcnt(0) lgkmcnt(0)
+	flat_store_dwordx4 v[20:21], v[2:5]
+	s_or_b64 exec, exec, s[40:41]
+	s_and_saveexec_b64 s[40:41], s[0:1]
+	s_cbranch_execz .LBB27_63
+.LBB27_67:
+	v_lshl_add_u64 v[20:21], v[22:23], 4, s[24:25]
+	s_waitcnt vmcnt(0) lgkmcnt(0)
+	flat_store_dwordx4 v[20:21], v[6:9]
+	s_or_b64 exec, exec, s[40:41]
+	s_and_saveexec_b64 s[0:1], s[8:9]
+	s_cbranch_execz .LBB27_64
diff --git a/profiles/direct_stream/loops_before_double_sum_w8.s b/profiles/direct_stream/loops_before_double_sum_w8.s
--- /dev/null
+++ b/profiles/direct_stream/loops_before_double_sum_w8.s
@@ -0,0 +1,536 @@
+
+.LBB34_19:
+	v_lshlrev_b64 v[32:33], 4, v[2:3]
+	v_lshl_add_u64 v[4:5], s[8:9], 0, v[32:33]
+	v_lshl_add_u64 v[8:9], s[10:11], 0, v[32:33]
+	v_lshl_add_u64 v[12:13], s[12:13], 0, v[32:33]
+	v_lshl_add_u64 v[16:17], s[14:15], 0, v[32:33]
+	v_lshl_add_u64 v[20:21], s[16:17], 0, v[32:33]
+	v_lshl_add_u64 v[24:25], s[18:19], 0, v[32:33]
+	v_lshl_add_u64 v[28:29], s[20:21], 0, v[32:33]
+	v_lshl_add_u64 v[38:39], s[22:23], 0, v[32:33]
+	flat_load_dwordx4 v[4:7], v[4:5] nt
+	s_nop 0
+	flat_load_dwordx4 v[8:11], v[8:9] nt
+	s_nop 0
+	flat_load_dwordx4 v[12:15], v[12:13] nt
+	s_nop 0
+	flat_load_dwordx4 v[16:19], v[16:17] nt
+	s_nop 0
+	flat_load_dwordx4 v[20:23], v[20:21] nt
+	s_nop 0
+	flat_load_dwordx4 v[24:27], v[24:25] nt
+	s_nop 0
+	flat_load_dwordx4 v[28:31], v[28:29] nt
+	s_nop 0
+	flat_load_dwordx4 v[38:41], v[38:39] nt
+	v_lshl_add_u64 v[2:3], v[2:3], 0, s[50:51]
+	v_cmp_le_u64_e32 vcc, s[42:43], v[2:3]
+	v_lshl_add_u64 v[32:33], s[46:47], 0, v[32:33]
+	s_or_b64 s[48:49], vcc, s[48:49]
+	s_waitcnt vmcnt(0) lgkmcnt(0)
+	v_add_f64 v[4:5], v[8:9], v[4:5]
+	v_add_f64 v[6:7], v[10:11], v[6:7]
+	v_add_f64 v[4:5], v[12:13], v[4:5]
+	v_add_f64 v[6:7], v[14:15], v[6:7]
+	v_add_f64 v[4:5], v[16:17], v[4:5]
+	v_add_f64 v[6:7], v[18:19], v[6:7]
+	v_add_f64 v[4:5], v[20:21], v[4:5]
+	v_add_f64 v[6:7], v[22:23], v[6:7]
+	v_add_f64 v[4:5], v[24:25], v[4:5]
+	v_add_f64 v[6:7], v[26:27], v[6:7]
+	v_add_f64 v[4:5], v[28:29], v[4:5]
+	v_add_f64 v[6:7], v[30:31], v[6:7]
+	v_add_f64 v[4:5], v[38:39], v[4:5]
+	v_add_f64 v[6:7], v[40:41], v[6:7]
+	flat_store_dwordx4 v[32:33], v[4:7]
+	s_andn2_b64 exec, exec, s[48:49]
+	s_cbranch_execnz .LBB34_19
+
+.LBB34_41:
+	s_or_b64 exec, exec, s[4:5]
+	s_mov_b64 s[4:5], 0x200
+	v_lshl_add_u64 v[36:37], v[36:37], 0, s[4:5]
+	v_cmp_le_u64_e32 vcc, s[30:31], v[36:37]
+	s_or_b64 s[94:95], vcc, s[94:95]
+	s_andn2_b64 exec, exec, s[94:95]
+	s_cbranch_execz .LBB34_74
+.LBB34_42:
+	v_cmp_gt_u64_e32 vcc, s[66:67], v[36:37]
+	s_and_b64 s[96:97], s[68:69], vcc
+	s_and_saveexec_b64 s[6:7], s[96:97]
+	s_cbranch_execz .LBB34_44
+	s_load_dwordx2 s[4:5], s[24:25], 0x80
+	s_waitcnt vmcnt(0) lgkmcnt(0)
+	v_lshl_add_u64 v[2:3], v[36:37], 4, s[4:5]
+	flat_load_dwordx4 v[2:5], v[2:3] nt
+.LBB34_44:
+	s_or_b64 exec, exec, s[6:7]
+	v_cmp_gt_u64_e32 vcc, s[70:71], v[36:37]
+	s_and_b64 s[98:99], s[60:61], vcc
+	s_and_saveexec_b64 s[6:7], s[98:99]
+	s_cbranch_execz .LBB34_46
+	s_load_dwordx2 s[4:5], s[24:25], 0x88
+	s_lshl_b64 s[14:15], s[26:27], 4
+	s_waitcnt lgkmcnt(0)
+	s_add_u32 s4, s4, s14
+	s_addc_u32 s5, s5, s15
+	s_waitcnt vmcnt(0)
+	v_lshl_add_u64 v[6:7], v[36:37], 4, s[4:5]
+	flat_load_dwordx4 v[6:9], v[6:7] nt
+.LBB34_46:
+	s_or_b64 exec, exec, s[6:7]
+	v_cmp_gt_u64_e32 vcc, s[72:73], v[36:37]
+	s_and_b64 s[34:35], s[54:55], vcc
+	s_and_saveexec_b64 s[6:7], s[34:35]
+	s_cbranch_execz .LBB34_48
+	s_load_dwordx2 s[4:5], s[24:25], 0x90
+	s_lshl_b64 s[14:15], s[28:29], 4
+	s_waitcnt lgkmcnt(0)
+	s_add_u32 s4, s4, s14
+	s_addc_u32 s5, s5, s15
+	s_waitcnt vmcnt(0)
+	v_lshl_add_u64 v[10:11], v[36:37], 4, s[4:5]
+	flat_load_dwordx4 v[10:13], v[10:11] nt
+.LBB34_48:
+	s_or_b64 exec, exec, s[6:7]
+	v_cmp_gt_u64_e32 vcc, s[74:75], v[36:37]
+	s_and_b64 s[6:7], s[48:49], vcc
+	s_and_saveexec_b64 s[14:15], s[6:7]
+	s_cbranch_execz .LBB34_50
+	s_load_dwordx2 s[4:5], s[24:25], 0x98
+	s_waitcnt lgkmcnt(0)
+	s_add_u32 s4, s4, s84
+	s_addc_u32 s5, s5, s85
+	s_waitcnt vmcnt(0)
+	v_lshl_add_u64 v[14:15], v[36:37], 4, s[4:5]
+	flat_load_dwordx4 v[14:17], v[14:15] nt
+.LBB34_50:
+	s_or_b64 exec, exec, s[14:15]
+	v_cmp_gt_u64_e32 vcc, s[76:77], v[36:37]
+	s_and_b64 s[14:15], s[42:43], vcc
+	s_and_saveexec_b64 s[20:21], s[14:15]
+	s_cbranch_execz .LBB34_52
+	s_load_dwordx2 s[4:5], s[24:25], 0xa0
+	s_waitcnt lgkmcnt(0)
+	s_add_u32 s4, s4, s86
+	s_addc_u32 s5, s5, s87
+	s_waitcnt vmcnt(0)
+	v_lshl_add_u64 v[18:19], v[36:37], 4, s[4:5]
+	flat_load_dwordx4 v[18:21], v[18:19] nt
+.LBB34_52:
+	s_or_b64 exec, exec, s[20:21]
+	v_cmp_gt_u64_e32 vcc, s[78:79], v[36:37]
+	s_and_b64 s[20:21], s[36:37], vcc
+	s_and_saveexec_b64 s[38:39], s[20:21]
+	s_cbranch_execz .LBB34_54
+	s_load_dwordx2 s[4:5], s[24:25], 0xa8
+	s_waitcnt lgkmcnt(0)
+	s_add_u32 s4, s4, s88
+	s_addc_u32 s5, s5, s89
+	s_waitcnt vmcnt(0)
+	v_lshl_add_u64 v[22:23], v[36:37], 4, s[4:5]
+	flat_load_dwordx4 v[22:25], v[22:23] nt
+.LBB34_54:
+	s_or_b64 exec, exec, s[38:39]
+	v_cmp_gt_u64_e32 vcc, s[80:81], v[36:37]
+	s_and_b64 s[38:39], s[18:19], vcc
+	s_and_saveexec_b64 vcc, s[38:39]
+	s_cbranch_execz .LBB34_56
+	s_load_dwordx2 s[4:5], s[24:25], 0xb0
+	s_waitcnt lgkmcnt(0)
+	s_add_u32 s4, s4, s90
+	s_addc_u32 s5, s5, s91
+	s_waitcnt vmcnt(0)
+	v_lshl_add_u64 v[26:27], v[36:37], 4, s[4:5]
+	flat_load_dwordx4 v[26:29], v[26:27] nt
+.LBB34_56:
+	s_or_b64 exec, exec, vcc
+	v_cmp_gt_u64_e32 vcc, s[82:83], v[36:37]
+	s_and_b64 vcc, s[12:13], vcc
+	s_and_saveexec_b64 s[4:5], vcc
+	s_cbranch_execnz .LBB34_65
+	s_or_b64 exec, exec, s[4:5]
+	s_waitcnt lgkmcnt(0)
+	v_lshl_add_u64 v[38:39], v[36:37], 4, s[0:1]
+	s_and_saveexec_b64 s[4:5], s[96:97]
+	s_cbranch_execnz .LBB34_66
+.LBB34_58:
+	s_or_b64 exec, exec, s[4:5]
+	s_and_saveexec_b64 s[4:5], s[98:99]
+	s_cbranch_execnz .LBB34_67
+.LBB34_59:
+	s_or_b64 exec, exec, s[4:5]
+	s_and_saveexec_b64 s[4:5], s[34:35]
+	s_cbranch_execnz .LBB34_68
+.LBB34_60:
+	s_or_b64 exec, exec, s[4:5]
+	s_and_saveexec_b64 s[4:5], s[6:7]
+	s_cbranch_execnz .LBB34_69
+.LBB34_61:
+	s_or_b64 exec, exec, s[4:5]
+	s_and_saveexec_b64 s[4:5], s[14:15]
+	s_cbranch_execnz .LBB34_70
+.LBB34_62:
+	s_or_b64 exec, exec, s[4:5]
+	s_and_saveexec_b64 s[4:5], s[20:21]
+	s_cbranch_execnz .LBB34_71
+.LBB34_63:
+	s_or_b64 exec, exec, s[4:5]
+	s_and_saveexec_b64 s[4:5], s[38:39]
+	s_cbranch_execnz .LBB34_72
+.LBB34_64:
+	s_or_b64 exec, exec, s[4:5]
+	s_and_saveexec_b64 s[4:5], vcc
+	s_cbranch_execz .LBB34_41
+
+.LBB34_58:
+	s_or_b64 exec, exec, s[4:5]
+	s_and_saveexec_b64 s[4:5], s[98:99]
+	s_cbranch_execnz .LBB34_67
+.LBB34_59:
+	s_or_b64 exec, exec, s[4:5]
+	s_and_saveexec_b64 s[4:5], s[34:35]
+	s_cbranch_execnz .LBB34_68
+.LBB34_60:
+	s_or_b64 exec, exec, s[4:5]
+	s_and_saveexec_b64 s[4:5], s[6:7]
+	s_cbranch_execnz .LBB34_69
+.LBB34_61:
+	s_or_b64 exec, exec, s[4:5]
+	s_and_saveexec_b64 s[4:5], s[14:15]
+	s_cbranch_execnz .LBB34_70
+.LBB34_62:
+	s_or_b64 exec, exec, s[4:5]
+	s_and_saveexec_b64 s[4:5], s[20:21]
+	s_cbranch_execnz .LBB34_71
+.LBB34_63:
+	s_or_b64 exec, exec, s[4:5]
+	s_and_saveexec_b64 s[4:5], s[38:39]
+	s_cbranch_execnz .LBB34_72
+.LBB34_64:
+	s_or_b64 exec, exec, s[4:5]
+	s_and_saveexec_b64 s[4:5], vcc
+	s_cbranch_execz .LBB34_41
+	s_branch .LBB34_73
+.LBB34_65:
+	s_load_dwordx2 s[44:45], s[24:25], 0xb8
+	s_waitcnt lgkmcnt(0)
+	s_add_u32 s44, s44, s92
+	s_addc_u32 s45, s45, s93
+	s_waitcnt vmcnt(0)
+	v_lshl_add_u64 v[30:31], v[36:37], 4, s[44:45]
+	flat_load_dwordx4 v[30:33], v[30:31] nt
+	s_or_b64 exec, exec, s[4:5]
+	v_lshl_add_u64 v[38:39], v[36:37], 4, s[0:1]
+	s_and_saveexec_b64 s[4:5], s[96:97]
+	s_cbranch_execz .LBB34_58
+
+.LBB34_59:
+	s_or_b64 exec, exec, s[4:5]
+	s_and_saveexec_b64 s[4:5], s[34:35]
+	s_cbranch_execnz .LBB34_68
+.LBB34_60:
+	s_or_b64 exec, exec, s[4:5]
+	s_and_saveexec_b64 s[4:5], s[6:7]
+	s_cbranch_execnz .LBB34_69
+.LBB34_61:
+	s_or_b64 exec, exec, s[4:5]
+	s_and_saveexec_b64 s[4:5], s[14:15]
+	s_cbranch_execnz .LBB34_70
+.LBB34_62:
+	s_or_b64 exec, exec, s[4:5]
+	s_and_saveexec_b64 s[4:5], s[20:21]
+	s_cbranch_execnz .LBB34_71
+.LBB34_63:
+	s_or_b64 exec, exec, s[4:5]
+	s_and_saveexec_b64 s[4:5], s[38:39]
+	s_cbranch_execnz .LBB34_72
+.LBB34_64:
+	s_or_b64 exec, exec, s[4:5]
+	s_and_saveexec_b64 s[4:5], vcc
+	s_cbranch_execz .LBB34_41
+	s_branch .LBB34_73
+.LBB34_65:
+	s_load_dwordx2 s[44:45], s[24:25], 0xb8
+	s_waitcnt lgkmcnt(0)
+	s_add_u32 s44, s44, s92
+	s_addc_u32 s45, s45, s93
+	s_waitcnt vmcnt(0)
+	v_lshl_add_u64 v[30:31], v[36:37], 4, s[44:45]
+	flat_load_dwordx4 v[30:33], v[30:31] nt
+	s_or_b64 exec, exec, s[4:5]
+	v_lshl_add_u64 v[38:39], v[36:37], 4, s[0:1]
+	s_and_saveexec_b64 s[4:5], s[96:97]
+	s_cbranch_execz .LBB34_58
+.LBB34_66:
+	s_waitcnt vmcnt(0)
+	flat_store_dwordx4 v[38:39], v[2:5]
+	s_or_b64 exec, exec, s[4:5]
+	s_and_saveexec_b64 s[4:5], s[98:99]
+	s_cbranch_execz .LBB34_59
+
+.LBB34_60:
+	s_or_b64 exec, exec, s[4:5]
+	s_and_saveexec_b64 s[4:5], s[6:7]
+	s_cbranch_execnz .LBB34_69
+.LBB34_61:
+	s_or_b64 exec, exec, s[4:5]
+	s_and_saveexec_b64 s[4:5], s[14:15]
+	s_cbranch_execnz .LBB34_70
+.LBB34_62:
+	s_or_b64 exec, exec, s[4:5]
+	s_and_saveexec_b64 s[4:5], s[20:21]
+	s_cbranch_execnz .LBB34_71
+.LBB34_63:
+	s_or_b64 exec, exec, s[4:5]
+	s_and_saveexec_b64 s[4:5], s[38:39]
+	s_cbranch_execnz .LBB34_72
+.LBB34_64:
+	s_or_b64 exec, exec, s[4:5]
+	s_and_saveexec_b64 s[4:5], vcc
+	s_cbranch_execz .LBB34_41
+	s_branch .LBB34_73
+.LBB34_65:
+	s_load_dwordx2 s[44:45], s[24:25], 0xb8
+	s_waitcnt lgkmcnt(0)
+	s_add_u32 s44, s44, s92
+	s_addc_u32 s45, s45, s93
+	s_waitcnt vmcnt(0)
+	v_lshl_add_u64 v[30:31], v[36:37], 4, s[44:45]
+	flat_load_dwordx4 v[30:33], v[30:31] nt
+	s_or_b64 exec, exec, s[4:5]
+	v_lshl_add_u64 v[38:39], v[36:37], 4, s[0:1]
+	s_and_saveexec_b64 s[4:5], s[96:97]
+	s_cbranch_execz .LBB34_58
+.LBB34_66:
+	s_waitcnt vmcnt(0)
+	flat_store_dwordx4 v[38:39], v[2:5]
+	s_or_b64 exec, exec, s[4:5]
+	s_and_saveexec_b64 s[4:5], s[98:99]
+	s_cbranch_execz .LBB34_59
+.LBB34_67:
+	v_lshl_add_u64 v[40:41], s[26:27], 4, v[38:39]
+	s_waitcnt vmcnt(0)
+	flat_store_dwordx4 v[40:41], v[6:9]
+	s_or_b64 exec, exec, s[4:5]
+	s_and_saveexec_b64 s[4:5], s[34:35]
+	s_cbranch_execz .LBB34_60
+
+.LBB34_61:
+	s_or_b64 exec, exec, s[4:5]
+	s_and_saveexec_b64 s[4:5], s[14:15]
+	s_cbranch_execnz .LBB34_70
+.LBB34_62:
+	s_or_b64 exec, exec, s[4:5]
+	s_and_saveexec_b64 s[4:5], s[20:21]
+	s_cbranch_execnz .LBB34_71
+.LBB34_63:
+	s_or_b64 exec, exec, s[4:5]
+	s_and_saveexec_b64 s[4:5], s[38:39]
+	s_cbranch_execnz .LBB34_72
+.LBB34_64:
+	s_or_b64 exec, exec, s[4:5]
+	s_and_saveexec_b64 s[4:5], vcc
+	s_cbranch_execz .LBB34_41
+	s_branch .LBB34_73
+.LBB34_65:
+	s_load_dwordx2 s[44:45], s[24:25], 0xb8
+	s_waitcnt lgkmcnt(0)
+	s_add_u32 s44, s44, s92
+	s_addc_u32 s45, s45, s93
+	s_waitcnt vmcnt(0)
+	v_lshl_add_u64 v[30:31], v[36:37], 4, s[44:45]
+	flat_load_dwordx4 v[30:33], v[30:31] nt
+	s_or_b64 exec, exec, s[4:5]
+	v_lshl_add_u64 v[38:39], v[36:37], 4, s[0:1]
+	s_and_saveexec_b64 s[4:5], s[96:97]
+	s_cbranch_execz .LBB34_58
+.LBB34_66:
+	s_waitcnt vmcnt(0)
+	flat_store_dwordx4 v[38:39], v[2:5]
+	s_or_b64 exec, exec, s[4:5]
+	s_and_saveexec_b64 s[4:5], s[98:99]
+	s_cbranch_execz .LBB34_59
+.LBB34_67:
+	v_lshl_add_u64 v[40:41], s[26:27], 4, v[38:39]
+	s_waitcnt vmcnt(0)
+	flat_store_dwordx4 v[40:41], v[6:9]
+	s_or_b64 exec, exec, s[4:5]
+	s_and_saveexec_b64 s[4:5], s[34:35]
+	s_cbranch_execz .LBB34_60
+.LBB34_68:
+	v_lshl_add_u64 v[40:41], s[28:29], 4, v[38:39]
+	s_waitcnt vmcnt(0)
+	flat_store_dwordx4 v[40:41], v[10:13]
+	s_or_b64 exec, exec, s[4:5]
+	s_and_saveexec_b64 s[4:5], s[6:7]
+	s_cbranch_execz .LBB34_61
+
+.LBB34_62:
+	s_or_b64 exec, exec, s[4:5]
+	s_and_saveexec_b64 s[4:5], s[20:21]
+	s_cbranch_execnz .LBB34_71
+.LBB34_63:
+	s_or_b64 exec, exec, s[4:5]
+	s_and_saveexec_b64 s[4:5], s[38:39]
+	s_cbranch_execnz .LBB34_72
+.LBB34_64:
+	s_or_b64 exec, exec, s[4:5]
+	s_and_saveexec_b64 s[4:5], vcc
+	s_cbranch_execz .LBB34_41
+	s_branch .LBB34_73
+.LBB34_65:
+	s_load_dwordx2 s[44:45], s[24:25], 0xb8
+	s_waitcnt lgkmcnt(0)
+	s_add_u32 s44, s44, s92
+	s_addc_u32 s45, s45, s93
+	s_waitcnt vmcnt(0)
+	v_lshl_add_u64 v[30:31], v[36:37], 4, s[44:45]
+	flat_load_dwordx4 v[30:33], v[30:31] nt
+	s_or_b64 exec, exec, s[4:5]
+	v_lshl_add_u64 v[38:39], v[36:37], 4, s[0:1]
+	s_and_saveexec_b64 s[4:5], s[96:97]
+	s_cbranch_execz .LBB34_58
+.LBB34_66:
+	s_waitcnt vmcnt(0)
+	flat_store_dwordx4 v[38:39], v[2:5]
+	s_or_b64 exec, exec, s[4:5]
+	s_and_saveexec_b64 s[4:5], s[98:99]
+	s_cbranch_execz .LBB34_59
+.LBB34_67:
+	v_lshl_add_u64 v[40:41], s[26:27], 4, v[38:39]
+	s_waitcnt vmcnt(0)
+	flat_store_dwordx4 v[40:41], v[6:9]
+	s_or_b64 exec, exec, s[4:5]
+	s_and_saveexec_b64 s[4:5], s[34:35]
+	s_cbranch_execz .LBB34_60
+.LBB34_68:
+	v_lshl_add_u64 v[40:41], s[28:29], 4, v[38:39]
+	s_waitcnt vmcnt(0)
+	flat_store_dwordx4 v[40:41], v[10:13]
+	s_or_b64 exec, exec, s[4:5]
+	s_and_saveexec_b64 s[4:5], s[6:7]
+	s_cbranch_execz .LBB34_61
+.LBB34_69:
+	v_lshl_add_u64 v[40:41], v[38:39], 0, s[84:85]
+	s_waitcnt vmcnt(0)
+	flat_store_dwordx4 v[40:41], v[14:17]
+	s_or_b64 exec, exec, s[4:5]
+	s_and_saveexec_b64 s[4:5], s[14:15]
+	s_cbranch_execz .LBB34_62
+
+.LBB34_63:
+	s_or_b64 exec, exec, s[4:5]
+	s_and_saveexec_b64 s[4:5], s[38:39]
+	s_cbranch_execnz .LBB34_72
+.LBB34_64:
+	s_or_b64 exec, exec, s[4:5]
+	s_and_saveexec_b64 s[4:5], vcc
+	s_cbranch_execz .LBB34_41
+	s_branch .LBB34_73
+.LBB34_65:
+	s_load_dwordx2 s[44:45], s[24:25], 0xb8
+	s_waitcnt lgkmcnt(0)
+	s_add_u32 s44, s44, s92
+	s_addc_u32 s45, s45, s93
+	s_waitcnt vmcnt(0)
+	v_lshl_add_u64 v[30:31], v[36:37], 4, s[44:45]
+	flat_load_dwordx4 v[30:33], v[30:31] nt
+	s_or_b64 exec, exec, s[4:5]
+	v_lshl_add_u64 v[38:39], v[36:37], 4, s[0:1]
+	s_and_saveexec_b64 s[4:5], s[96:97]
+	s_cbranch_execz .LBB34_58
+.LBB34_66:
+	s_waitcnt vmcnt(0)
+	flat_store_dwordx4 v[38:39], v[2:5]
+	s_or_b64 exec, exec, s[4:5]
+	s_and_saveexec_b64 s[4:5], s[98:99]
+	s_cbranch_execz .LBB34_59
+.LBB34_67:
+	v_lshl_add_u64 v[40:41], s[26:27], 4, v[38:39]
+	s_waitcnt vmcnt(0)
+	flat_store_dwordx4 v[40:41], v[6:9]
+	s_or_b64 exec, exec, s[4:5]
+	s_and_saveexec_b64 s[4:5], s[34:35]
+	s_cbranch_execz .LBB34_60
+.LBB34_68:
+	v_lshl_add_u64 v[40:41], s[28:29], 4, v[38:39]
+	s_waitcnt vmcnt(0)
+	flat_store_dwordx4 v[40:41], v[10:13]
+	s_or_b64 exec, exec, s[4:5]
+	s_and_saveexec_b64 s[4:5], s[6:7]
+	s_cbranch_execz .LBB34_61
+.LBB34_69:
+	v_lshl_add_u64 v[40:41], v[38:39], 0, s[84:85]
+	s_waitcnt vmcnt(0)
+	flat_store_dwordx4 v[40:41], v[14:17]
+	s_or_b64 exec, exec, s[4:5]
+	s_and_saveexec_b64 s[4:5], s[14:15]
+	s_cbranch_execz .LBB34_62
+.LBB34_70:
+	v_lshl_add_u64 v[40:41], v[38:39], 0, s[86:87]
+	s_waitcnt vmcnt(0)
+	flat_store_dwordx4 v[40:41], v[18:21]
+	s_or_b64 exec, exec, s[4:5]
+	s_and_saveexec_b64 s[4:5], s[20:21]
+	s_cbranch_execz .LBB34_63
+
+.LBB34_64:
+	s_or_b64 exec, exec, s[4:5]
+	s_and_saveexec_b64 s[4:5], vcc
+	s_cbranch_execz .LBB34_41
+	s_branch .LBB34_73
+.LBB34_65:
+	s_load_dwordx2 s[44:45], s[24:25], 0xb8
+	s_waitcnt lgkmcnt(0)
+	s_add_u32 s44, s44, s92
+	s_addc_u32 s45, s45, s93
+	s_waitcnt vmcnt(0)
+	v_lshl_add_u64 v[30:31], v[36:37], 4, s[44:45]
+	flat_load_dwordx4 v[30:33], v[30:31] nt
+	s_or_b64 exec, exec, s[4:5]
+	v_lshl_add_u64 v[38:39], v[36:37], 4, s[0:1]
+	s_and_saveexec_b64 s[4:5], s[96:97]
+	s_cbranch_execz .LBB34_58
+.LBB34_66:
+	s_waitcnt vmcnt(0)
+	flat_store_dwordx4 v[38:39], v[2:5]
+	s_or_b64 exec, exec, s[4:5]
+	s_and_saveexec_b64 s[4:5], s[98:99]
+	s_cbranch_execz .LBB34_59
+.LBB34_67:
+	v_lshl_add_u64 v[40:41], s[26:27], 4, v[38:39]
+	s_waitcnt vmcnt(0)
+	flat_store_dwordx4 v[40:41], v[6:9]
+	s_or_b64 exec, exec, s[4:5]
+	s_and_saveexec_b64 s[4:5], s[34:35]
+	s_cbranch_execz .LBB34_60
+.LBB34_68:
+	v_lshl_add_u64 v[40:41], s[28:29], 4, v[38:39]
+	s_waitcnt vmcnt(0)
+	flat_store_dwordx4 v[40:41], v[10:13]
+	s_or_b64 exec, exec, s[4:5]
+	s_and_saveexec_b64 s[4:5], s[6:7]
+	s_cbranch_execz .LBB34_61
+.LBB34_69:
+	v_lshl_add_u64 v[40:41], v[38:39], 0, s[84:85]
+	s_waitcnt vmcnt(0)
+	flat_store_dwordx4 v[40:41], v[14:17]
+	s_or_b64 exec, exec, s[4:5]
+	s_and_saveexec_b64 s[4:5], s[14:15]
+	s_cbranch_execz .LBB34_62
+.LBB34_70:
+	v_lshl_add_u64 v[40:41], v[38:39], 0, s[86:87]
+	s_waitcnt vmcnt(0)
+	flat_store_dwordx4 v[40:41], v[18:21]
+	s_or_b64 exec, exec, s[4:5]
+	s_and_saveexec_b64 s[4:5], s[20:21]
+	s_cbranch_execz .LBB34_63
+.LBB34_71:
+	v_lshl_add_u64 v[40:41], v[38:39], 0, s[88:89]
+	s_waitcnt vmcnt(0)
+	flat_store_dwordx4 v[40:41], v[22:25]
+	s_or_b64 exec, exec, s[4:5]
+	s_and_saveexec_b64 s[4:5], s[38:39]
+	s_cbranch_execz .LBB34_64
```

After: 7368 GB/s (median of 4 runs). Within noise of the previous version (+0.1%).
